# cocowy1/PPMStereo

Hardware: AMD Instinct MI355X
Metric: disparity-px/s (higher is better)
Workload: dtype bf16; 1 GPU; BASELINE config 2: T=5 clip at 320x512, iters=10, hot path only (3-scale cascade from encoder outputs: corr pyramid build + lookup, QAM pick, pick-and-play memory attention, ConvGRU3D update, heads, convex upsample, test_mode=True as PPMStereo.forward_batch_test calls it: predictions[-1] is the output, so the mask head, the convex upsampling and the full-resolution resize run only where their resu; T=5, H=320, W=512, iters=10, parallelism=replicas x1

## Files before the change

### include/ppms.h

```cpp
#ifndef PPMS_H
#define PPMS_H
#include <stdint.h>

#ifdef __cplusplus
extern "C" {
#endif

#define PPMS_OK 0
#define PPMS_EINVAL (-1)
#define PPMS_ELAUNCH (-2)
#define PPMS_ENODEV (-3)

#define PPMS_ABI_VERSION 4

int ppms_version(void);
const char* ppms_last_error(void);
int ppms_device_info(char* name, int name_cap, int* cu_count, int* clock_mhz);

int ppms_corr_build(const float* fmap1, const float* fmap2, float* const pyr[5], int B, int C, int H, int W, void* stream);

int ppms_corr_lookup(const float* const pyr[4], const float* flow, int flow_nhwc, float* out_nchw, void* out_hi, void* out_lo,
                     int out_ld, void* flow_sp_hi, void* flow_sp_lo, int flow_sp_ld, int B, int H, int W, void* stream);

typedef struct ppms_sp {
    void* hi;
    void* lo;
    int32_t ld;
    int32_t c;
} ppms_sp;

enum {
    PPMS_EPI_STORE = 0,
    PPMS_EPI_RESID = 1,
    PPMS_EPI_RH = 2,
    PPMS_EPI_GRU = 3,
    PPMS_EPI_ADDF32 = 4
};
enum { PPMS_ACT_NONE = 0, PPMS_ACT_RELU = 1, PPMS_ACT_GELU = 2, PPMS_ACT_SIGMOID = 3, PPMS_ACT_TANH = 4, PPMS_ACT_ELU1 = 5  };

typedef struct ppms_epilogue {
    int32_t kind, act;
    float scale;
    int32_t n_valid;
    ppms_sp out_sp;
    float* out_f32;
    int32_t out_f32_ld;
    int32_t vt_f16;
    void* out_vt;
    ppms_sp aux_sp;
    const float* aux_f32;
    int32_t aux_f32_ld;
    int32_t pre_f32_ld;
    const float* pre_f32;
} ppms_epilogue;

typedef struct ppms_conv {
    ppms_sp seg[2];
    int32_t nseg;
    int32_t groups;
    const void* w;
    const float* bias;
    int32_t T, H, W;
    int32_t kt, kh, kw;
    int32_t M;
    int32_t m_split;
    int32_t t_halo;
    int32_t lo_zero_from;
    ppms_epilogue epi[2];
} ppms_conv;

int ppms_conv_gemm2(const ppms_conv* desc, const ppms_conv* dev_desc, int wm_hint, void* stream);
int ppms_conv_gemm2_slices(const ppms_conv* desc);
int64_t ppms_conv_gemm2_slice_workspace_bytes(const ppms_conv* desc, int nslice);
int ppms_conv_gemm2_sliced(const ppms_conv* desc, const ppms_conv* dev_desc, int nslice, void* workspace, void* stream);
int ppms_conv_gemm2_ysweep_slices(const ppms_conv* desc);
int ppms_conv_gemm2_ysweep(const ppms_conv* desc, const ppms_conv* dev_desc, int nslice, void* workspace, void* stream);
int ppms_conv_gemm5_applicable(const ppms_conv* desc);
int ppms_conv_gemm5(const ppms_conv* desc, const ppms_conv* dev_desc, int nbt, void* stream);
int ppms_conv_gemm5_slices(const ppms_conv* desc);
int ppms_conv_gemm5_sliced(const ppms_conv* desc, const ppms_conv* dev_desc, int nbt, int nslice, void* workspace, void* stream);
int ppms_conv_gemm6_applicable(const ppms_conv* desc);
int ppms_conv_gemm6(const ppms_conv* desc, const ppms_conv* dev_desc, void* stream);
int ppms_gemm1_applicable(const ppms_conv* desc);
int ppms_gemm1(const ppms_conv* desc, const ppms_conv* dev_desc, int cb_hint, void* stream);
int ppms_conv_stream_applicable(const ppms_conv* desc);
int ppms_conv_stream(const ppms_conv* desc, const ppms_conv* dev_desc, int hint, void* stream);
int ppms_struct_sizes(int* sp, int* epilogue, int* conv);

int ppms_dwconv_gelu(ppms_sp x, ppms_sp y, const float* w, const float* b, int k, int BT, int H, int W, void* stream);
int ppms_flow_patch7(const float* flow_nhwc, ppms_sp patch, int BT, int H, int W, void* stream);
int ppms_unc_tail(ppms_sp x, const float* w, float bias, float* unc, float* partial, int BT, int HW, void* stream);

int ppms_nchw_to_sp(const float* src, ppms_sp dst, int BT, int C, int HW, void* stream);
int ppms_sp_to_nchw(ppms_sp src, float* dst, int BT, int C, int HW, void* stream);
int ppms_nchw_to_nhwc(const float* src, float* dst, int dst_ld, int BT, int C, int HW, void* stream);
int ppms_nhwc_to_nchw(const float* src, int src_ld, float* dst, int BT, int C, int HW, void* stream);
int ppms_f32_to_sp(const float* src, int src_ld, ppms_sp dst, int64_t pixels, void* stream);
int ppms_sp_to_f32(ppms_sp src, float* dst, int dst_ld, int64_t pixels, void* stream);

int ppms_tap_gather_sum(const float* y, int y_ld, const float* bias, float* out, int out_ld, float* accum, int accum_ld, int cout, int kt, int kh,
                        int kw, int T, int H, int W, int t_halo, void* stream);
int ppms_flow_add(float* flow_nhwc, const float* dflow, int dflow_ld, int64_t pixels, void* stream);
int ppms_convex_upsample(const float* flow_nhwc, const float* mask, int mask_ld, float* out, int BT, int H, int W, void* stream);
int ppms_convex_upsample_3d(const float* flow_nhwc, const float* mask, int mask_ld, float* out, int T, int H, int W, int t_halo, void* stream);
int ppms_bilinear(const float* src, float* dst, int N, int C, int H, int W, int OH, int OW, int align_corners, float mul, void* stream);

int ppms_sp_resize_blend(ppms_sp src, ppms_sp dst, int N, int H, int W, int OH, int OW, float a, float b, void* stream);

int ppms_avgpool(const float* src, float* dst, int planes, int H, int W, int k, void* stream);
int ppms_axpby(const float* x, const float* y, float* out, float a, float b, int64_t period, int64_t n, void* stream);
int ppms_ctx_mix(const float* fmap, const float* ctx, float* net, float* inp, int N, int HW, void* stream);

int ppms_img_s2d(const float* img_nchw, ppms_sp dst, int N, int C, int H, int W, int k, void* stream);
int ppms_sp_s2d(ppms_sp src, ppms_sp dst, int N, int H, int W, void* stream);
int64_t ppms_instnorm_workspace_bytes(int N, int HW, int C);
int ppms_instnorm_stats(const float* x, int ld, int N, int HW, int C, float eps, float* stats, void* workspace, void* stream);
int ppms_instnorm_apply(const float* x, int ld, const float* stats, ppms_sp res, int relu, ppms_sp out, int N, int HW, int C, void* stream);

int ppms_dwconv(ppms_sp x, float* y, int ldy, const float* w, const float* b, int k, int N, int H, int W, void* stream);
int ppms_layernorm_any(const float* x, int ld, const float* w, const float* b, float eps, ppms_sp out, int64_t pixels, int C, void* stream);
int64_t ppms_grn_workspace_bytes(int N, int HW, int C);
int ppms_grn(const float* x, int ld, const float* gamma, const float* beta, ppms_sp out, int N, int HW, int C, void* workspace, void* stream);
int ppms_sp_upsample2(ppms_sp src, ppms_sp dst, int N, int H, int W, void* stream);

int ppms_qk_similarity(const float* q, const float* k, int ld, float* pooled, float* sim, int T, int H, int W, void* stream);
int ppms_qk_pool(const float* q, const float* k, int ld, float* pooled, int T, int H, int W, void* stream);
int ppms_qk_cos(const float* pooled, float* sim, int T, int cells, void* stream);
int ppms_qam_select(const float* sim, float* strive, const float* conf_partial, int nblk, int HW, int32_t* sel, float* shat,
                    float* score, int T, void* stream);
int ppms_attn_prep_q(const float* q, int ld, const float* pe, void* qb, int T, int n, void* stream);
int ppms_attn_prep_k(const float* key, int ld, const float* pe, const int32_t* sel, const float* shat, void* kb, int T, int ksel,
                     int n, void* stream);
enum { PPMS_ATTN_P_BF16 = 0, PPMS_ATTN_P_FP16 = 1 };
int ppms_mem_attn(const void* qb, const void* kb, const void* vt, const int32_t* sel, int ksel, float scale, const float* beta,
                  ppms_sp mf, ppms_sp mfg, void* out_bf16, int T, int n, void* split_ws, int frames_per_workgroup, int p_format, void* stream);
int64_t ppms_mem_attn_workspace_bytes(int T, int ksel, int n);

int ppms_pwchain(const void* dev_params, int64_t pixels, void* stream);
int ppms_pwchain_param_bytes(void);

int ppms_time_attn(ppms_sp x, const float* ln_w, const float* ln_b, ppms_sp out, int T, int n, int heads, void* stream);
int ppms_layernorm(const float* x, int ld, const float* w, const float* b, ppms_sp resid, ppms_sp out, int64_t pixels, int C, void* stream);
int64_t ppms_linear_attention_workspace_floats(int T, int n, int heads, int dh);
int ppms_linear_attention(const float* Q, int ldq, const float* K, int ldk, const float* V, int ldv, float* kv_ws, ppms_sp out, int T, int n,
                          int heads, int dh, void* stream);

#ifdef __cplusplus
}
#endif
#endif
```

### ppmstereo_amd/_lib.py

```python
from __future__ import annotations

import ctypes as C
import os
from typing import Optional

import torch

from . import build as _build

c_void_p, c_int, c_float, c_int64 = C.c_void_p, C.c_int, C.c_float, C.c_int64

EPI_STORE, EPI_RESID, EPI_RH, EPI_GRU, EPI_ADDF32 = range(5)
ATTN_P_BF16, ATTN_P_FP16 = 0, 1
ACT_NONE, ACT_RELU, ACT_GELU, ACT_SIGMOID, ACT_TANH, ACT_ELU1 = range(6)


def vt_image(v: torch.Tensor, p_format: int) -> torch.Tensor:
    b = v.to(torch.bfloat16)
    if p_format == ATTN_P_BF16:
        return b.contiguous()
    return b.float().clamp(-65504.0, 65504.0).to(torch.float16).contiguous().view(torch.bfloat16)


def vt_values(vt: torch.Tensor, p_format: int) -> torch.Tensor:
    return vt.float() if p_format == ATTN_P_BF16 else vt.view(torch.float16).float()


class SP(C.Structure):
    _fields_ = [("hi", c_void_p), ("lo", c_void_p), ("ld", C.c_int32), ("c", C.c_int32)]


class Epilogue(C.Structure):
    _fields_ = [("kind", C.c_int32), ("act", C.c_int32), ("scale", c_float), ("n_valid", C.c_int32),
                ("out_sp", SP), ("out_f32", c_void_p), ("out_f32_ld", C.c_int32), ("vt_f16", C.c_int32), ("out_vt", c_void_p),
                ("aux_sp", SP), ("aux_f32", c_void_p), ("aux_f32_ld", C.c_int32), ("pre_f32_ld", C.c_int32),
                ("pre_f32", c_void_p)]


class Conv(C.Structure):
    _fields_ = [("seg", SP * 2), ("nseg", C.c_int32), ("groups", C.c_int32), ("w", c_void_p), ("bias", c_void_p),
                ("T", C.c_int32), ("H", C.c_int32), ("W", C.c_int32),
                ("kt", C.c_int32), ("kh", C.c_int32), ("kw", C.c_int32),
                ("M", C.c_int32), ("m_split", C.c_int32), ("t_halo", C.c_int32), ("lo_zero_from", C.c_int32), ("epi", Epilogue * 2)]


class ChainLayer(C.Structure):
    _fields_ = [("w", c_void_p), ("bias", c_void_p), ("post_s", c_void_p), ("post_t", c_void_p),
                ("M", C.c_int32), ("n_valid", C.c_int32), ("resid", C.c_int32)]


class ChainParams(C.Structure):
    _fields_ = [("inp", SP), ("out", SP), ("layer", ChainLayer * 3), ("nlayers", C.c_int32), ("P", C.c_int64)]


_SIGS = {
    "ppms_version": (c_int, []),
    "ppms_last_error": (C.c_char_p, []),
    "ppms_device_info": (c_int, [C.c_char_p, c_int, C.POINTER(c_int), C.POINTER(c_int)]),
    "ppms_corr_build": (c_int, [c_void_p, c_void_p, C.POINTER(c_void_p), c_int, c_int, c_int, c_int, c_void_p]),
    "ppms_corr_lookup": (c_int, [C.POINTER(c_void_p), c_void_p, c_int, c_void_p, c_void_p, c_void_p, c_int, c_void_p, c_void_p,
                                 c_int, c_int, c_int, c_int, c_void_p]),
    "ppms_conv_gemm2": (c_int, [C.POINTER(Conv), c_void_p, c_int, c_void_p]),
    "ppms_conv_gemm2_slices": (c_int, [C.POINTER(Conv)]),
    "ppms_conv_gemm2_slice_workspace_bytes": (C.c_int64, [C.POINTER(Conv), c_int]),
    "ppms_conv_gemm2_sliced": (c_int, [C.POINTER(Conv), c_void_p, c_int, c_void_p, c_void_p]),
    "ppms_conv_gemm2_ysweep_slices": (c_int, [C.POINTER(Conv)]),
    "ppms_conv_gemm2_ysweep": (c_int, [C.POINTER(Conv), c_void_p, c_int, c_void_p, c_void_p]),
    "ppms_gemm1_applicable": (c_int, [C.POINTER(Conv)]),
    "ppms_gemm1": (c_int, [C.POINTER(Conv), c_void_p, c_int, c_void_p]),
    "ppms_conv_stream_applicable": (c_int, [C.POINTER(Conv)]),
    "ppms_conv_stream": (c_int, [C.POINTER(Conv), c_void_p, c_int, c_void_p]),
    "ppms_conv_gemm5_applicable": (c_int, [C.POINTER(Conv)]),
    "ppms_conv_gemm5": (c_int, [C.POINTER(Conv), c_void_p, c_int, c_void_p]),
    "ppms_conv_gemm6_applicable": (c_int, [C.POINTER(Conv)]),
    "ppms_conv_gemm6": (c_int, [C.POINTER(Conv), c_void_p, c_void_p]),
    "ppms_conv_gemm5_slices": (c_int, [C.POINTER(Conv)]),
    "ppms_conv_gemm5_sliced": (c_int, [C.POINTER(Conv), c_void_p, c_int, c_int, c_void_p, c_void_p]),
    "ppms_struct_sizes": (c_int, [C.POINTER(c_int), C.POINTER(c_int), C.POINTER(c_int)]),
    "ppms_dwconv_gelu": (c_int, [SP, SP, c_void_p, c_void_p, c_int, c_int, c_int, c_int, c_void_p]),
    "ppms_flow_patch7": (c_int, [c_void_p, SP, c_int, c_int, c_int, c_void_p]),
    "ppms_unc_tail": (c_int, [SP, c_void_p, c_float, c_void_p, c_void_p, c_int, c_int, c_void_p]),
    "ppms_nchw_to_sp": (c_int, [c_void_p, SP, c_int, c_int, c_int, c_void_p]),
    "ppms_sp_to_nchw": (c_int, [SP, c_void_p, c_int, c_int, c_int, c_void_p]),
    "ppms_nchw_to_nhwc": (c_int, [c_void_p, c_void_p, c_int, c_int, c_int, c_int, c_void_p]),
    "ppms_nhwc_to_nchw": (c_int, [c_void_p, c_int, c_void_p, c_int, c_int, c_int, c_void_p]),
    "ppms_f32_to_sp": (c_int, [c_void_p, c_int, SP, c_int64, c_void_p]),
    "ppms_sp_to_f32": (c_int, [SP, c_void_p, c_int, c_int64, c_void_p]),
    "ppms_tap_gather_sum": (c_int, [c_void_p, c_int, c_void_p, c_void_p, c_int, c_void_p, c_int, c_int, c_int, c_int, c_int, c_int, c_int, c_int, c_int, c_void_p]),
    "ppms_flow_add": (c_int, [c_void_p, c_void_p, c_int, c_int64, c_void_p]),
    "ppms_convex_upsample": (c_int, [c_void_p, c_void_p, c_int, c_void_p, c_int, c_int, c_int, c_void_p]),
    "ppms_convex_upsample_3d": (c_int, [c_void_p, c_void_p, c_int, c_void_p, c_int, c_int, c_int, c_int, c_void_p]),
    "ppms_bilinear": (c_int, [c_void_p, c_void_p, c_int, c_int, c_int, c_int, c_int, c_int, c_int, c_float, c_void_p]),
    "ppms_sp_resize_blend": (c_int, [SP, SP, c_int, c_int, c_int, c_int, c_int, c_float, c_float, c_void_p]),
    "ppms_avgpool": (c_int, [c_void_p, c_void_p, c_int, c_int, c_int, c_int, c_void_p]),
    "ppms_axpby": (c_int, [c_void_p, c_void_p, c_void_p, c_float, c_float, c_int64, c_int64, c_void_p]),
    "ppms_ctx_mix": (c_int, [c_void_p, c_void_p, c_void_p, c_void_p, c_int, c_int, c_void_p]),
    "ppms_img_s2d": (c_int, [c_void_p, SP, c_int, c_int, c_int, c_int, c_int, c_void_p]),
    "ppms_dwconv": (c_int, [SP, c_void_p, c_int, c_void_p, c_void_p, c_int, c_int, c_int, c_int, c_void_p]),
    "ppms_layernorm_any": (c_int, [c_void_p, c_int, c_void_p, c_void_p, c_float, SP, c_int64, c_int, c_void_p]),
    "ppms_grn_workspace_bytes": (c_int64, [c_int, c_int, c_int]),
    "ppms_grn": (c_int, [c_void_p, c_int, c_void_p, c_void_p, SP, c_int, c_int, c_int, c_void_p, c_void_p]),
    "ppms_sp_upsample2": (c_int, [SP, SP, c_int, c_int, c_int, c_void_p]),
    "ppms_sp_s2d": (c_int, [SP, SP, c_int, c_int, c_int, c_void_p]),
    "ppms_instnorm_workspace_bytes": (c_int64, [c_int, c_int, c_int]),
    "ppms_instnorm_stats": (c_int, [c_void_p, c_int, c_int, c_int, c_int, C.c_float, c_void_p, c_void_p, c_void_p]),
    "ppms_instnorm_apply": (c_int, [c_void_p, c_int, c_void_p, SP, c_int, SP, c_int, c_int, c_int, c_void_p]),
    "ppms_qk_similarity": (c_int, [c_void_p, c_void_p, c_int, c_void_p, c_void_p, c_int, c_int, c_int, c_void_p]),
    "ppms_qk_pool": (c_int, [c_void_p, c_void_p, c_int, c_void_p, c_int, c_int, c_int, c_void_p]),
    "ppms_qk_cos": (c_int, [c_void_p, c_void_p, c_int, c_int, c_void_p]),
    "ppms_qam_select": (c_int, [c_void_p, c_void_p, c_void_p, c_int, c_int, c_void_p, c_void_p, c_void_p, c_int, c_void_p]),
    "ppms_attn_prep_q": (c_int, [c_void_p, c_int, c_void_p, c_void_p, c_int, c_int, c_void_p]),
    "ppms_attn_prep_k": (c_int, [c_void_p, c_int, c_void_p, c_void_p, c_void_p, c_void_p, c_int, c_int, c_int, c_void_p]),
    "ppms_pwchain": (c_int, [c_void_p, c_int64, c_void_p]),
    "ppms_pwchain_param_bytes": (c_int, []),
    "ppms_time_attn": (c_int, [SP, c_void_p, c_void_p, SP, c_int, c_int, c_int, c_void_p]),
    "ppms_layernorm": (c_int, [c_void_p, c_int, c_void_p, c_void_p, SP, SP, c_int64, c_int, c_void_p]),
    "ppms_linear_attention_workspace_floats": (c_int64, [c_int, c_int, c_int, c_int]),
    "ppms_linear_attention": (c_int, [c_void_p, c_int, c_void_p, c_int, c_void_p, c_int, c_void_p, SP, c_int, c_int, c_int, c_int, c_void_p]),
    "ppms_mem_attn": (c_int, [c_void_p, c_void_p, c_void_p, c_void_p, c_int, c_float, c_void_p, SP, SP, c_void_p, c_int, c_int, c_void_p, c_int, c_int, c_void_p]),
    "ppms_mem_attn_workspace_bytes": (c_int64, [c_int, c_int, c_int]),
}
EXPORTS = tuple(_SIGS)

_lib: Optional[C.CDLL] = None


def lib_path() -> str:
    return _build.LIB


def load() -> C.CDLL:
    global _lib
    if _lib is not None:
        return _lib
    try:
        path = _build.build(verbose=not os.path.exists(_build.LIB))
        lib = C.CDLL(path)
    except Exception as exc:
        raise RuntimeError(f"ppmstereo_amd: the HIP library libppms.so is missing and could not be built ({exc}); "
                           "there is no CPU fallback") from exc
    for name, (res, args) in _SIGS.items():
        fn = getattr(lib, name)
        fn.restype, fn.argtypes = res, args
    if lib.ppms_version() != 4:
        raise RuntimeError("ppmstereo_amd: libppms.so ABI version mismatch")
    a, b, c = c_int(), c_int(), c_int()
    lib.ppms_struct_sizes(C.byref(a), C.byref(b), C.byref(c))
    if (a.value, b.value, c.value) != (C.sizeof(SP), C.sizeof(Epilogue), C.sizeof(Conv)):
        raise RuntimeError("ppmstereo_amd: ctypes struct layout differs from include/ppms.h")
    if lib.ppms_pwchain_param_bytes() != C.sizeof(ChainParams):
        raise RuntimeError("ppmstereo_amd: ChainParams layout differs from pwchain.hip")
    _lib = lib
    return lib


def check(rc: int) -> None:
    if rc != 0:
        raise RuntimeError("libppms: " + load().ppms_last_error().decode())


def stream_ptr() -> int:
    return torch.cuda.current_stream().cuda_stream


def require_gpu(*tensors: torch.Tensor) -> None:
    for t in tensors:
        if t is not None and not t.is_cuda:
            raise RuntimeError("ppmstereo_amd ops run on the GPU only (got a CPU tensor); there is no CPU fallback")


def ptr(t: Optional[torch.Tensor]) -> Optional[int]:
    return None if t is None else t.data_ptr()


class SPTensor:

    def __init__(self, pixels: int, channels: int, device, zero: bool = True, before: int = 0, after: int = 0):
        alloc = torch.zeros if zero else torch.empty
        self.data = alloc((2, before + pixels + after, channels), dtype=torch.bfloat16, device=device)
        self.pixels, self.channels, self.before, self.after = pixels, channels, before, after

    def view(self, c0: int = 0, c: Optional[int] = None, all_rows: bool = False) -> SP:
        c = self.channels - c0 if c is None else c
        assert 0 <= c0 and c0 + c <= self.channels
        total = self.before + self.pixels + self.after
        base = self.data.data_ptr() + (0 if all_rows else self.before) * self.channels * 2
        plane = total * self.channels * 2
        return SP(base + c0 * 2, base + plane + c0 * 2, self.channels, c)

    def own(self) -> torch.Tensor:
        return self.data[:, self.before:self.before + self.pixels]

    def to_f32(self, c0: int = 0, c: Optional[int] = None) -> torch.Tensor:
        c = self.channels - c0 if c is None else c
        d = self.own()
        return d[0, :, c0:c0 + c].float() + d[1, :, c0:c0 + c].float()

    def set_f32(self, x: torch.Tensor, c0: int = 0) -> None:
        hi = x.to(torch.bfloat16)
        lo = (x - hi.float()).to(torch.bfloat16)
        d = self.own()
        d[0, :, c0:c0 + x.shape[1]] = hi
        d[1, :, c0:c0 + x.shape[1]] = lo
```

### ppmstereo_amd/build.py

```python
from __future__ import annotations

import fcntl
import hashlib
import os
import shutil
import subprocess
import sys
import tempfile

HERE = os.path.dirname(os.path.abspath(__file__))
ROOT = os.path.dirname(HERE)
CSRC = os.path.join(HERE, "csrc")
LIB = os.path.join(HERE, "libppms.so")
STAMP = LIB + ".stamp"
LOCK = LIB + ".lock"
SOURCES = ["corr.hip", "conv_gemm2.hip", "conv_gemm5.hip", "conv_gemm6.hip", "gemm1.hip", "conv_stream.hip", "small_ops.hip", "encoder_ops.hip", "mem_attn.hip", "attn16.hip", "pwchain.hip"]
HEADERS = ["common.h", "corr_lookup.h", "conv_epilogue.h", "conv5_asm.h", "conv6_asm.h", "attn64_asm.h", os.path.join("..", "..", "include", "ppms.h")]
COMMON = ["--offload-arch=gfx950", "-O3", "-std=c++17", "-fPIC", "-ffp-contract=off", "-I" + os.path.join(ROOT, "include"), "-I" + CSRC]
NO_PK = ["-Xclang", "-target-feature", "-Xclang", "-packed-fp32-ops"]
EXTRA = [x for x in os.environ.get("PPMS_BUILD_DEFINES", "").split() if x]
PACKED_FP32_SOURCES: tuple = tuple(x for x in os.environ.get("PPMS_BUILD_PACKED_FP32", "").split(",") if x)
FLAGS = COMMON + NO_PK + EXTRA


def _digest() -> str:
    h = hashlib.sha256(" ".join(x.replace(ROOT, "$ROOT") for x in FLAGS + list(PACKED_FP32_SOURCES)).encode())
    for f in SOURCES + HEADERS:
        with open(os.path.join(CSRC, f), "rb") as fh:
            h.update(os.path.basename(f).encode() + fh.read())
    return h.hexdigest()


def _fresh(dig: str) -> bool:
    try:
        return os.path.exists(LIB) and open(STAMP).read() == dig
    except OSError:
        return False


def build(force: bool = False, verbose: bool = True) -> str:
    dig = _digest()
    if not force and _fresh(dig):
        return LIB
    hipcc = os.environ.get("HIPCC", "/opt/rocm/bin/hipcc")
    noise = "'-packed-fp32-ops' is not a recognized feature for this target (ignoring feature)"

    def run(cmd):
        if verbose:
            print("[ppmstereo_amd.build]", " ".join(cmd), file=sys.stderr)
        res = subprocess.run(cmd, stderr=subprocess.PIPE, text=True)
        err = "\n".join(ln for ln in res.stderr.splitlines() if noise not in ln)
        if err.strip():
            print(err, file=sys.stderr)
        if res.returncode != 0:
            raise subprocess.CalledProcessError(res.returncode, cmd)

    with open(LOCK, "w") as lock:
        fcntl.flock(lock, fcntl.LOCK_EX)
        try:
            if not force and _fresh(dig):
                return LIB
            tmp = tempfile.mkdtemp(prefix="_build_", dir=HERE)
            try:
                objs = []
                procs = []
                for src in SOURCES:
                    obj = os.path.join(tmp, src.replace(".hip", ".o"))
                    cmd = [hipcc] + (COMMON + EXTRA if src in PACKED_FP32_SOURCES else FLAGS) + ["-c", os.path.join(CSRC, src), "-o", obj]
                    if verbose:
                        print("[ppmstereo_amd.build]", " ".join(cmd), file=sys.stderr)
                    procs.append((cmd, subprocess.Popen(cmd, stderr=subprocess.PIPE, text=True)))
                    objs.append(obj)
                for cmd, pr in procs:
                    _, err = pr.communicate()
                    err = "\n".join(ln for ln in err.splitlines() if noise not in ln)
                    if err.strip():
                        print(err, file=sys.stderr)
                    if pr.returncode != 0:
                        raise subprocess.CalledProcessError(pr.returncode, cmd)
                out = os.path.join(tmp, "libppms.so")
                run([hipcc, "--offload-arch=gfx950", "-shared", "-fPIC"] + objs + ["-o", out])
                stamp = os.path.join(tmp, "stamp")
                with open(stamp, "w") as fh:
                    fh.write(dig)
                if os.path.exists(STAMP):
                    os.remove(STAMP)
                os.replace(out, LIB)
                os.replace(stamp, STAMP)
            finally:
                shutil.rmtree(tmp, ignore_errors=True)
        finally:
            fcntl.flock(lock, fcntl.LOCK_UN)
    return LIB


if __name__ == "__main__":
    print(build(force="--force" in sys.argv))
```

### ppmstereo_amd/csrc/pwchain.hip

```cpp
#include "common.h"

namespace {

constexpr int TP = 128;
constexpr int ROWB = 64;
constexpr int ACT_PLANE = TP * ROWB;
constexpr int ACT_BUF = 4 * ACT_PLANE;
constexpr int W_BLK = 2 * 2 * 64 * 64;

__device__ __forceinline__ int swzp(int row, int chunk) { return row * 64 + ((chunk ^ ((row >> 2) & 3)) << 4); }

struct Layer {
    const void* w;
    const float* bias;
    const float* post_s;
    const float* post_t;
    int M;
    int n_valid;
    int resid;
};

struct ChainParams {
    ppms_sp in, out;
    Layer layer[3];
    int nlayers;
    int64_t P;
};

__global__ __launch_bounds__(256) void pwchain_kernel(const ChainParams* __restrict__ cp) {
    extern __shared__ __attribute__((aligned(16))) char smem[];
    const ChainParams& c = *cp;
    char* bufX = smem;
    char* bufA = smem + ACT_BUF;
    char* wsm = smem + 2 * ACT_BUF;
    const int tid = threadIdx.x, lane = tid & 63, wave = tid >> 6;
    const int r = lane & 31, h = lane >> 5;
    const int64_t p0 = (int64_t)blockIdx.x * TP;

    for (int q = tid; q < TP * 8; q += 256) {
        const int px = q >> 3, ch = q & 7;
        const int64_t pix = p0 + px;
        u32x4 vh = {0, 0, 0, 0}, vl = {0, 0, 0, 0};
        if (pix < c.P) {
            vh = gload16((const bf16_t*)c.in.hi + pix * c.in.ld + ch * 8);
            vl = gload16((const bf16_t*)c.in.lo + pix * c.in.ld + ch * 8);
        }
        const int off = (ch >> 2) * 2 * ACT_PLANE + swzp(px, ch & 3);
        *(u32x4*)(bufX + off) = vh;
        *(u32x4*)(bufX + ACT_PLANE + off) = vl;
    }
    u32x4 wreg[4];
    auto load_w = [&](int l, int mblk) __attribute__((always_inline)) {
        const Layer& Lw = c.layer[l];
        const int mbs = Lw.M / 64;
#pragma unroll
        for (int i = 0; i < 4; ++i) {
            const int q = tid + i * 256;
            const int ks = q >> 9, rem = q & 511;
            wreg[i] = gload16((const char*)Lw.w + ((int64_t)(ks * mbs + mblk) * 512 + rem) * 16);
        }
    };
    load_w(0, 0);
    const char* src = bufX;
    for (int l = 0; l < c.nlayers; ++l) {
        const Layer& L = c.layer[l];
        const bool last = (l == c.nlayers - 1);
        char* dst = (src == bufX) ? bufA : bufX;
        const int mblocks = L.M / 64;
        for (int mblk = 0; mblk < mblocks; ++mblk) {
            __syncthreads();
#pragma unroll
            for (int i = 0; i < 4; ++i) *(u32x4*)(wsm + (tid + i * 256) * 16) = wreg[i];
            if (mblk + 1 < mblocks)
                load_w(l, mblk + 1);
            else if (l + 1 < c.nlayers)
                load_w(l + 1, 0);
            __syncthreads();
            f32x16 acc[2];
            acc[0] = (f32x16){0};
            acc[1] = (f32x16){0};
#pragma unroll
            for (int ks = 0; ks < 2; ++ks) {
#pragma unroll
                for (int k16 = 0; k16 < 2; ++k16) {
                    const int boff = ks * 2 * ACT_PLANE + swzp(wave * 32 + r, 2 * k16 + h);
                    const bf16x8 bh = *(const bf16x8*)(src + boff);
                    const bf16x8 bl = *(const bf16x8*)(src + ACT_PLANE + boff);
#pragma unroll
                    for (int mb = 0; mb < 2; ++mb) {
                        const int aoff = ks * 8192 + swzp(mb * 32 + r, 2 * k16 + h);
                        const bf16x8 ah = *(const bf16x8*)(wsm + aoff);
                        const bf16x8 al = *(const bf16x8*)(wsm + 4096 + aoff);
                        acc[mb] = __builtin_amdgcn_mfma_f32_32x32x16_bf16(al, bh, acc[mb], 0, 0, 0);
                        acc[mb] = __builtin_amdgcn_mfma_f32_32x32x16_bf16(ah, bl, acc[mb], 0, 0, 0);
                        acc[mb] = __builtin_amdgcn_mfma_f32_32x32x16_bf16(ah, bh, acc[mb], 0, 0, 0);
                    }
                }
            }
            const int px = wave * 32 + r;
            const int64_t pix = p0 + px;
#pragma unroll
            for (int mb = 0; mb < 2; ++mb)
#pragma unroll
                for (int g = 0; g < 4; ++g) {
                    const int cl = mb * 32 + 8 * g + 4 * h;
                    const int cg = mblk * 64 + cl;
                    const f32x4 b4 = gld<f32x4>(L.bias + cg);
                    float y[4];
#pragma unroll
                    for (int j = 0; j < 4; ++j) y[j] = acc[mb][4 * g + j] + b4[j];
                    if (L.resid) {
                        const int xo = (cl >> 5) * 2 * ACT_PLANE + swzp(px, (cl & 31) >> 3) + (cl & 7) * 2;
                        const bf16x4 xh = *(const bf16x4*)(bufX + xo), xl = *(const bf16x4*)(bufX + ACT_PLANE + xo);
#pragma unroll
                        for (int j = 0; j < 4; ++j) y[j] += join_bf16(xh[j], xl[j]);
                    }
#pragma unroll
                    for (int j = 0; j < 4; ++j) y[j] = gelu_erf(y[j]);
                    if (L.post_s != nullptr) {
                        const f32x4 s4 = gld<f32x4>(L.post_s + cg), t4 = gld<f32x4>(L.post_t + cg);
#pragma unroll
                        for (int j = 0; j < 4; ++j) y[j] = gelu_erf(y[j] + (y[j] * s4[j] + t4[j]));
                    }
                    bf16x4 oh, ol;
#pragma unroll
                    for (int j = 0; j < 4; ++j) {
                        bf16_t hh = (bf16_t)0.0f, ll = (bf16_t)0.0f;
                        if (cg + j < L.n_valid) split_bf16(y[j], hh, ll);
                        oh[j] = hh;
                        ol[j] = ll;
                    }
                    {
                        const int xo = (cl >> 5) * 2 * ACT_PLANE + swzp(px, (cl & 31) >> 3) + (cl & 7) * 2;
                        *(bf16x4*)(dst + xo) = oh;
                        *(bf16x4*)(dst + ACT_PLANE + xo) = ol;
                    }
                }
            if (last) {
                __syncthreads();
                for (int qd = tid; qd < TP * 16; qd += 256) {
                    const int opx = qd >> 4, plane = (qd >> 3) & 1, ch = qd & 7;
                    const int64_t opix = p0 + opx;
                    const int ocg = mblk * 64 + ch * 8;
                    if (opix < c.P && ocg < L.n_valid) {
                        const u32x4 v = *(const u32x4*)(dst + (ch >> 2) * 2 * ACT_PLANE + plane * ACT_PLANE + swzp(opx, ch & 3));
                        bf16_t* op = (bf16_t*)(plane ? c.out.lo : c.out.hi) + opix * c.out.ld + ocg;
                        if (ocg + 8 <= L.n_valid) {
                            gstore16(op, v);
                        } else {
                            const bf16_t* e = (const bf16_t*)&v;
                            for (int j = 0; j < 8; ++j)
                                if (ocg + j < L.n_valid) gst<bf16_t>(op + j, e[j]);
                        }
                    }
                }
            }
        }
        src = dst;
    }
}

constexpr int TP32 = 32;
constexpr int ACT32_PLANE = TP32 * ROWB;
constexpr int ACT32_BUF = 4 * ACT32_PLANE;
constexpr int W32_MAX = 4 * W_BLK;

__global__ __launch_bounds__(256) void pwchain32_kernel(const ChainParams* __restrict__ cp) {
    extern __shared__ __attribute__((aligned(16))) char smem[];
    const ChainParams& c = *cp;
    char* bufX = smem;
    char* bufA = smem + ACT32_BUF;
    char* wsm = smem + 2 * ACT32_BUF;
    const int tid = threadIdx.x, lane = tid & 63, wave = tid >> 6;
    const int r = lane & 31, h = lane >> 5;
    const int64_t p0 = (int64_t)blockIdx.x * TP32;
    {
        const int px = tid >> 3, ch = tid & 7;
        const int64_t pix = p0 + px;
        u32x4 vh = {0, 0, 0, 0}, vl = {0, 0, 0, 0};
        if (pix < c.P) {
            vh = gload16((const bf16_t*)c.in.hi + pix * c.in.ld + ch * 8);
            vl = gload16((const bf16_t*)c.in.lo + pix * c.in.ld + ch * 8);
        }
        const int off = (ch >> 2) * 2 * ACT32_PLANE + swzp(px, ch & 3);
        *(u32x4*)(bufX + off) = vh;
        *(u32x4*)(bufX + ACT32_PLANE + off) = vl;
    }
    u32x4 wreg[16];
    auto load_w = [&](int l) __attribute__((always_inline)) {
        const Layer& Lw = c.layer[l];
        const int mbs = Lw.M / 64;
#pragma unroll
        for (int mblk = 0; mblk < 4; ++mblk)
            if (mblk < mbs) {
#pragma unroll
                for (int i = 0; i < 4; ++i) {
                    const int q = tid + i * 256;
                    const int ks = q >> 9, rem = q & 511;
                    wreg[mblk * 4 + i] = gload16((const char*)Lw.w + ((int64_t)(ks * mbs + mblk) * 512 + rem) * 16);
                }
            }
    };
    load_w(0);
    const char* src = bufX;
    for (int l = 0; l < c.nlayers; ++l) {
        const Layer& L = c.layer[l];
        const bool last = (l == c.nlayers - 1);
        char* dst = (src == bufX) ? bufA : bufX;
        const int mbs = L.M / 64, nrb = L.M / 32;
        __syncthreads();
#pragma unroll
        for (int mblk = 0; mblk < 4; ++mblk)
            if (mblk < mbs) {
#pragma unroll
                for (int i = 0; i < 4; ++i) *(u32x4*)(wsm + mblk * W_BLK + (tid + i * 256) * 16) = wreg[mblk * 4 + i];
            }
        if (l + 1 < c.nlayers) load_w(l + 1);
        __syncthreads();
        bf16x4 keep_h[2][4], keep_l[2][4];
#pragma unroll
        for (int it = 0; it < 2; ++it) {
            const int rb = wave + 4 * it;
            if (rb >= nrb) continue;
            const int mblk = rb >> 1, mb = rb & 1;
            f32x16 acc = (f32x16){0};
#pragma unroll
            for (int ks = 0; ks < 2; ++ks)
#pragma unroll
                for (int k16 = 0; k16 < 2; ++k16) {
                    const int boff = ks * 2 * ACT32_PLANE + swzp(r, 2 * k16 + h);
                    const bf16x8 bh = *(const bf16x8*)(src + boff), bl = *(const bf16x8*)(src + ACT32_PLANE + boff);
                    const int aoff = mblk * W_BLK + ks * 8192 + swzp(mb * 32 + r, 2 * k16 + h);
                    const bf16x8 ah = *(const bf16x8*)(wsm + aoff), al = *(const bf16x8*)(wsm + 4096 + aoff);
                    acc = __builtin_amdgcn_mfma_f32_32x32x16_bf16(al, bh, acc, 0, 0, 0);
                    acc = __builtin_amdgcn_mfma_f32_32x32x16_bf16(ah, bl, acc, 0, 0, 0);
                    acc = __builtin_amdgcn_mfma_f32_32x32x16_bf16(ah, bh, acc, 0, 0, 0);
                }
#pragma unroll
            for (int g = 0; g < 4; ++g) {
                const int cl = mb * 32 + 8 * g + 4 * h;
                const int cg = mblk * 64 + cl;
                const f32x4 b4 = gld<f32x4>(L.bias + cg);
                float y[4];
#pragma unroll
                for (int j = 0; j < 4; ++j) y[j] = acc[4 * g + j] + b4[j];
                const int xo = (cl >> 5) * 2 * ACT32_PLANE + swzp(r, (cl & 31) >> 3) + (cl & 7) * 2;
                if (L.resid) {
                    const bf16x4 xh = *(const bf16x4*)(bufX + xo), xl = *(const bf16x4*)(bufX + ACT32_PLANE + xo);
#pragma unroll
                    for (int j = 0; j < 4; ++j) y[j] += join_bf16(xh[j], xl[j]);
                }
#pragma unroll
                for (int j = 0; j < 4; ++j) y[j] = gelu_erf(y[j]);
                if (L.post_s != nullptr) {
                    const f32x4 s4 = gld<f32x4>(L.post_s + cg), t4 = gld<f32x4>(L.post_t + cg);
#pragma unroll
                    for (int j = 0; j < 4; ++j) y[j] = gelu_erf(y[j] + (y[j] * s4[j] + t4[j]));
                }
                bf16x4 oh, ol;
#pragma unroll
                for (int j = 0; j < 4; ++j) {
                    bf16_t hh = (bf16_t)0.0f, ll = (bf16_t)0.0f;
                    if (cg + j < L.n_valid) split_bf16(y[j], hh, ll);
                    oh[j] = hh;
                    ol[j] = ll;
                }
                if (last) {
                    keep_h[it][g] = oh;
                    keep_l[it][g] = ol;
                } else {
                    *(bf16x4*)(dst + xo) = oh;
                    *(bf16x4*)(dst + ACT32_PLANE + xo) = ol;
                }
            }
        }
        if (last) {
            __syncthreads();
            const int rowb = L.M * 2 + 16;
#pragma unroll
            for (int it = 0; it < 2; ++it) {
                const int rb = wave + 4 * it;
                if (rb >= nrb) continue;
#pragma unroll
                for (int g = 0; g < 4; ++g) {
                    const int cg = rb * 32 + 8 * g + 4 * h;
                    *(bf16x4*)(wsm + r * rowb + cg * 2) = keep_h[it][g];
                    *(bf16x4*)(wsm + TP32 * rowb + r * rowb + cg * 2) = keep_l[it][g];
                }
            }
            __syncthreads();
            const int cpr = L.M / 8;
            for (int qd = tid; qd < TP32 * 2 * cpr; qd += 256) {
                const int plane = qd / (TP32 * cpr), rem = qd - plane * TP32 * cpr;
                const int opx = rem / cpr, ch = rem - opx * cpr;
                const int64_t opix = p0 + opx;
                const int ocg = ch * 8;
                if (opix < c.P && ocg < L.n_valid) {
                    const u32x4 v = *(const u32x4*)(wsm + plane * TP32 * rowb + opx * rowb + ocg * 2);
                    bf16_t* op = (bf16_t*)(plane ? c.out.lo : c.out.hi) + opix * c.out.ld + ocg;
                    if (ocg + 8 <= L.n_valid) {
                        gstore16(op, v);
                    } else {
                        const bf16_t* e = (const bf16_t*)&v;
                        for (int j = 0; j < 8; ++j)
                            if (ocg + j < L.n_valid) gst<bf16_t>(op + j, e[j]);
                    }
                }
            }
        }
        src = dst;
    }
}

}

static int pwchain_launch(const void* dev_params, int64_t pixels, void* stream) {
    constexpr size_t lds = 2 * ACT_BUF + W_BLK;
    constexpr size_t lds32 = 2 * ACT32_BUF + W32_MAX;
    static ppms_device_once once;
    once.run([] {
        (void)hipFuncSetAttribute((const void*)pwchain_kernel, hipFuncAttributeMaxDynamicSharedMemorySize, (int)(2 * ACT_BUF + W_BLK));
        (void)hipFuncSetAttribute((const void*)pwchain32_kernel, hipFuncAttributeMaxDynamicSharedMemorySize, (int)(2 * ACT32_BUF + W32_MAX));
    });
    if (pixels <= 16384) {
        hipLaunchKernelGGL(pwchain32_kernel, dim3(ceil_div(pixels, TP32)), dim3(256), lds32, (hipStream_t)stream, (const ChainParams*)dev_params);
        return ppms_check_launch("pwchain");
    }
    hipLaunchKernelGGL(pwchain_kernel, dim3(ceil_div(pixels, TP)), dim3(256), lds, (hipStream_t)stream, (const ChainParams*)dev_params);
    return ppms_check_launch("pwchain");
}

extern "C" int ppms_pwchain(const void* dev_params, int64_t pixels, void* stream) {
    PPMS_REQUIRE(dev_params != nullptr && pixels > 0, "pwchain: bad arguments");
    return pwchain_launch(dev_params, pixels, stream);
}

extern "C" int ppms_pwchain_param_bytes(void) { return (int)sizeof(ChainParams); }
```

### ppmstereo_amd/engine.py

```python
from __future__ import annotations

import ctypes as C
import math
from typing import Dict, List, Optional

import torch

from . import _lib as L
from . import packing as _packing
from .convplan import (ALL_KERNELS, CONV2, CONV2_SWEPT, CONV6, KERNEL_TIMING, TUNING, ConvOp, PwChain, TimedCall,
                       attn_p_format, conv_desc, epilogue, pack_conv, plan_conv)

TOP_K = 5


def temporal_pe(T: int, channels: int) -> torch.Tensor:
    pos = torch.arange(T)
    pos = pos / pos[-1] * 1.0
    pos = pos.unsqueeze(1)
    div = 1.0 / (10000.0 ** (torch.arange(0, channels, 2).float() / channels))
    ang = pos * div
    pe = torch.zeros(T, channels)
    pe[:, 0::2] = torch.sin(ang)
    pe[:, 1::2] = torch.cos(ang)
    return pe


def softmax_scale(c: int = 128) -> float:
    return c ** -0.5 * math.log(2 * c, 12000)


class PackedBlock:

    def __init__(self, sd: Dict[str, torch.Tensor], device):
        g = lambda k: sd[k].detach().to(device=device, dtype=torch.float32)
        self.w: Dict[str, dict] = {}

        def put(name, weight, bias, segs, seg_pad=None, cout_map=None, m_pad=None, kernels=ALL_KERNELS):
            self.w[name] = pack_conv(weight, bias, segs, seg_pad, cout_map, m_pad, kernels)

        e = "encoder."
        put("init0", g(e + "init_conv.0.weight"), g(e + "init_conv.0.bias"), [128])
        put("init2", g(e + "init_conv.2.weight"), g(e + "init_conv.2.bias"), [64])
        c1 = e + "convc1."
        put("ffn1_0", g(c1 + "ffn1.0.weight"), g(c1 + "ffn1.0.bias"), [36], [64], kernels=(CONV2,))
        put("ffn1_2", g(c1 + "ffn1.2.weight"), g(c1 + "ffn1.2.bias"), [54], [64], kernels=(CONV2,))
        put("pw", g(c1 + "pw.weight"), g(c1 + "pw.bias"), [36], [64], kernels=(CONV2,))
        put("ffn2_0", g(c1 + "ffn2.0.weight"), g(c1 + "ffn2.0.bias"), [36], [64], kernels=(CONV2,))
        put("ffn2_2", g(c1 + "ffn2.2.weight"), g(c1 + "ffn2.2.bias"), [54], [64], kernels=(CONV2,))
        self.dw = []
        for i, k in ((0, 1), (1, 7)):
            w = torch.zeros(64, k * k, device=device)
            b = torch.zeros(64, device=device)
            w[:36] = g(c1 + f"conv_list.{i}.weight").reshape(36, k * k)
            b[:36] = g(c1 + f"conv_list.{i}.bias")
            self.dw.append((w.contiguous(), b.contiguous(), k))
        put("convc2", g(e + "convc2.weight"), g(e + "convc2.bias"), [256])
        wf1 = g(e + "convf1.weight").permute(0, 2, 3, 1).reshape(128, 98, 1, 1)
        put("convf1", wf1, g(e + "convf1.bias"), [98], [128])
        put("convf2", g(e + "convf2.weight"), g(e + "convf2.bias"), [128])
        put("final", g(e + "final_conv.weight"), g(e + "final_conv.bias"), [320], None, list(range(126)) + list(range(128, 192)), 192)
        put("to_v", g("aggregator.to_v.weight"), None, [128])
        put("unc0", g("uncertainty.0.weight"), g("uncertainty.0.bias"), [128, 128])
        self.unc2_w = g("uncertainty.2.weight").reshape(128).contiguous()
        self.unc2_b = float(sd["uncertainty.2.bias"].detach().float().cpu().item())
        gr = "gru."
        cat = lambda a, b: torch.cat([g(a), g(b)], 0)
        put("zr1_0", cat(gr + "convz1.0.weight", gr + "convr1.0.weight"), cat(gr + "convz1.0.bias", gr + "convr1.0.bias"), [128, 384])
        put("z1_2", g(gr + "convz1.2.weight"), g(gr + "convz1.2.bias"), [128])
        put("r1_2", g(gr + "convr1.2.weight"), g(gr + "convr1.2.bias"), [128])
        self.w["zr1_2"] = {CONV6: _packing.pack_conv6_grouped([g(gr + "convz1.2.weight"), g(gr + "convr1.2.weight")], [g(gr + "convz1.2.bias"), g(gr + "convr1.2.bias")], 128)}
        put("q1", g(gr + "convq1.weight"), g(gr + "convq1.bias"), [128, 384])
        for n in ("2", "3"):
            put("zr" + n, cat(gr + f"convz{n}.weight", gr + f"convr{n}.weight"), cat(gr + f"convz{n}.bias", gr + f"convr{n}.bias"), [128, 384])
            put("q" + n, g(gr + f"convq{n}.weight"), g(gr + f"convq{n}.bias"), [128, 384])
        self.hoist = "time_attn.temporal_fc.weight" not in sd
        if self.hoist:
            for name in ("zr1_0", "q1", "zr2", "q2", "zr3", "q3"):
                if name.startswith("zr"):
                    n_ = name[2:].replace("1_0", "1.0")
                    wt, bs = cat(gr + f"convz{n_}.weight", gr + f"convr{n_}.weight"), cat(gr + f"convz{n_}.bias", gr + f"convr{n_}.bias")
                else:
                    wt, bs = g(gr + f"convq{name[1:]}.weight"), g(gr + f"convq{name[1:]}.bias")
                w_h = torch.cat([wt[:, :128], wt[:, 256:]], 1).contiguous()
                put(name + "_i", wt[:, 128:256].contiguous(), bs, [128], kernels=ALL_KERNELS - {CONV2_SWEPT})
                put(name + "_h", w_h, None, [128, 256])
                beta = float(sd["aggregator.beta"].detach().double().reshape(-1)[0])
                wd = wt.double()
                w_x = torch.cat([wd[:, :128], wd[:, 256:384] + wd[:, 384:], beta * wd[:, 384:]], 1).float().contiguous()
                put(name + "_x", w_x, None, [128, 256])
        put("fh1", g("flow_head.conv1.weight"), g("flow_head.conv1.bias"), [128])
        w2 = g("flow_head.conv2.weight")
        put("fh2", w2.permute(2, 3, 4, 0, 1).reshape(54, 256, 1, 1, 1).contiguous(), None, [256])
        self.fh2_bias = g("flow_head.conv2.bias").contiguous()
        self.convex_3d = "mask_3d.0.weight" in sd
        mk = "mask_3d." if self.convex_3d else "mask_2d."
        put("m1", g(mk + "0.weight"), g(mk + "0.bias"), [128])
        put("m2", g(mk + "2.weight"), g(mk + "2.bias"), [256])
        self.mask_ch = 432 if self.convex_3d else 144
        self.beta = g("aggregator.beta").contiguous()
        self.attn = None
        if "time_attn.temporal_fc.weight" in sd:
            self.attn = {k: g(k) for k in sd if k.startswith("time_attn.") or k.startswith("space_attn.")}
            lin = lambda k: g(k)[:, :, None, None]
            ta, sa = "time_attn.", "space_attn.encoder_layer."
            w_fc, w_pj = g(ta + "temporal_fc.weight").double(), g(ta + "temporal_attn.proj.weight").double()
            w_ta = (w_fc @ w_pj).float().contiguous()
            b_ta = (w_fc @ g(ta + "temporal_attn.proj.bias").double() + g(ta + "temporal_fc.bias").double()).float().contiguous()
            put("ta_fc", w_ta[:, :, None, None], b_ta, [384])
            put("sa_qkv", torch.cat([lin(sa + "q_proj.weight"), lin(sa + "k_proj.weight"), lin(sa + "v_proj.weight")], 0), None, [384])
            put("sa_merge", lin(sa + "merge.weight"), None, [384])
            put("sa_mlp0", lin(sa + "mlp.0.weight"), None, [384, 384])
            put("sa_mlp2", lin(sa + "mlp.2.weight"), None, [768])
            self.ln = {k: (g(p_ + ".weight").contiguous(), g(p_ + ".bias").contiguous())
                       for k, p_ in (("ta", ta + "temporal_norm1"), ("n1", sa + "norm1"), ("n2", sa + "norm2"))}


class ScaleEngine:

    def __init__(self, pk: PackedBlock, T: int, h: int, w: int, device, shard=None):
        if shard is not None and shard.world == 1 and not getattr(shard, "force_comm", False):
            shard = None
        if shard is not None and T != shard.f:
            raise ValueError(f"sharded engine: {T} local frames, the shard holds {shard.f}")
        self.shard = shard
        self.Tg = Tg = T if shard is None else shard.T
        self.f0 = 0 if shard is None else shard.lo
        self.halo = 0 if shard is None else shard.HALO
        if Tg > 64:
            raise NotImplementedError("more than 64 frames per window")
        self.pk, self.T, self.h, self.w = pk, T, h, w
        self.n = n = h * w
        self.P = P = T * h * w
        self.dev = device
        self.ksel = min(TOP_K, Tg)
        hp = self.halo * n
        sp = lambda c: L.SPTensor(P, c, device, before=hp, after=hp)
        f32 = lambda *s: torch.zeros(*s, dtype=torch.float32, device=device)
        self.CORR, self.T1, self.C1, self.C2 = sp(64), sp(64), sp(64), sp(64)
        self.COR256, self.CF, self.PATCH, self.FLO1 = sp(256), [sp(320), sp(320)], sp(128), sp(128)
        self.X, self.VAL, self.U1 = sp(384), sp(128), sp(128)
        self.XA = sp(384) if pk.attn is not None else self.X
        if pk.attn is not None:
            self.XT, self.MSG, self.MSGN, self.H1 = sp(384), sp(384), sp(384), sp(768)
            self.O1 = L.SPTensor(P, 384, device, before=self.f0 * n, after=(Tg - self.f0 - T) * n)
            self.XG = self.X if shard is None else L.SPTensor(Tg * n, 384, device)
            self.QKF, self.VF, self.M2, self.M3 = f32(P, 768), f32(P, 384), f32(P, 384), f32(P, 384)
            self.KVWS = f32(int(L.load().ppms_linear_attention_workspace_floats(T, n, 8, 48)))
        self.Hb = [sp(128), sp(128), sp(128)]
        self.ZT, self.RT, self.RH, self.FH1, self.M1 = sp(128), sp(128), sp(128), sp(256), sp(256)
        self.Z, self.MASK, self.QK = f32(P, 128), f32(P, pk.mask_ch), f32(P, 256)
        self._FLOW_full, self._FH2Y_full = f32(P + 2 * hp, 2), f32(P + 2 * hp, 64)
        self.FLOW, self.FH2Y = self._FLOW_full[hp:hp + P], self._FH2Y_full[hp:hp + P]
        self.DFLOW = f32(P, 4)
        if pk.hoist:
            self.PRE = {k: torch.empty(P, m, dtype=torch.float32, device=device) for k, m in
                        (("zr1_0", 256), ("q1", 128), ("zr2", 256), ("q2", 128), ("zr3", 256), ("q3", 128))}
            self._pre_stream, self._ev_pre, self._pre_pending = torch.cuda.Stream(device=device), torch.cuda.Event(), False
        self.attn_p = attn_p_format()
        self.VT = torch.zeros(T, 128, n, dtype=torch.bfloat16, device=device)
        self.VTG = self.VT if shard is None else torch.zeros(Tg, 128, n, dtype=torch.bfloat16, device=device)
        self.KG = None if shard is None else f32(Tg * n, 128)
        self.QB = torch.zeros(T, n, 128, dtype=torch.bfloat16, device=device)
        self.KB = torch.zeros(T, self.ksel, n, 128, dtype=torch.bfloat16, device=device)
        self.ATT_WS = torch.empty(int(L.load().ppms_mem_attn_workspace_bytes(T, self.ksel, n)), dtype=torch.uint8, device=device)
        self.nblk = (n + 255) // 256
        self.UNC, self.PART = f32(P), f32(T, self.nblk)
        self.PARTG = self.PART if shard is None else f32(Tg, self.nblk)
        self.SIM, self.STRIVE, self.SCORE = f32(Tg, Tg), f32(Tg, Tg), f32(Tg, Tg)
        self.SEL = torch.zeros(Tg, 5, dtype=torch.int32, device=device)
        self.SHAT = f32(Tg, 5)
        self.cells = max(1, (h // 4) * (w // 4))
        self.POOL = f32(2, T, self.cells)
        self.POOLG = self.POOL if shard is None else f32(2, Tg, self.cells)
        self.PE = temporal_pe(Tg, 128).to(device)
        self.FLOW_OUT = f32(T, 2, 4 * h, 4 * w)
        self.scale = softmax_scale(128)
        self.parity = 0
        self.have_mhs = False
        self.lib = L.load()
        self._ev, self._ev_i = None, 0
        self._xa_halo = None
        self._x_hid = False
        self.hbm = {"corr_lookup": TimedCall(self._lookup), "attn_prep_k": TimedCall(self._prep_k), "convex_upsample": TimedCall(self._upsample)}
        self._side = torch.cuda.Stream(device=device)
        self._ev_fork, self._ev_join = torch.cuda.Event(), torch.cuda.Event()
        self._build_descriptors()

    def _halo_sp(self, tensors, k: int, async_op: bool = False):
        if self.shard is None:
            return None
        if isinstance(tensors, L.SPTensor):
            tensors = [tensors]
        fr = self.T + 2 * self.halo
        return self.shard.halo_many([(t.data[p].view(fr, self.n, t.channels), k) for t in tensors for p in (0, 1)], async_op)

    def _halo_f32(self, full: torch.Tensor, k: int):
        if self.shard is not None:
            self.shard.halo(full.view(self.T + 2 * self.halo, self.n, full.shape[1]), k)

    def _conv(self, packs, segs: List[L.SP], k3, epi0: L.Epilogue, epi1: Optional[L.Epilogue] = None, m_split: int = 0, keep=(),
              lo_zero_from: int = 0) -> ConvOp:
        d = conv_desc(segs, (self.T, self.h, self.w), k3, epi0, epi1, m_split, self.halo if k3[0] > 1 else 0, lo_zero_from)
        return plan_conv(d, self.pk.w[packs] if isinstance(packs, str) else packs, keep, device=self.dev)

    def _build_descriptors(self):
        E, X, H = epilogue, self.X, self.Hb
        k1, k3 = (1, 1, 1), (1, 3, 3)
        inp, mf, mfg = X.view(0, 128), X.view(128, 128), X.view(256, 128)
        self.op: Dict[str, object] = {}
        o = self.op
        self._qk_ops: Dict[int, ConvOp] = {}
        o["init0"] = self._conv("init0", [inp], k3, E(act=L.ACT_RELU, n_valid=64, out_sp=self.ZT.view(0, 64)))
        w = {k: self.pk.w[k][CONV2] for k in ("ffn1_0", "ffn1_2", "pw", "ffn2_0", "ffn2_2")}
        (w1, b1, _), (w7, b7, _) = self.pk.dw
        dw1 = (w1.reshape(64).contiguous(), b1)
        o["chainA"] = PwChain(self.CORR.view(), self.C2.view(), [(w["ffn1_0"], 54, False, None), (w["ffn1_2"], 36, True, dw1)], self.P, [dw1[0]],
                             device=self.dev)
        o["chainB"] = PwChain(self.C1.view(), self.COR256.view(), [(w["pw"], 36, True, None), (w["ffn2_0"], 54, False, None),
                                                                   (w["ffn2_2"], 256, False, None)], self.P, [], device=self.dev)
        o["dw7"] = TimedCall(lambda: L.check(self.lib.ppms_dwconv_gelu(self.C2.view(0, 40), self.C1.view(0, 40), w7.data_ptr(), b7.data_ptr(), 7,
                                                                        self.T, self.h, self.w, L.stream_ptr())))
        o["convf1"] = self._conv("convf1", [self.PATCH.view()], k1, E(act=L.ACT_RELU, n_valid=128, out_sp=self.FLO1.view()))
        for par in (0, 1):
            cf, cf_next = self.CF[par], self.CF[1 - par]
            o[f"init2_{par}"] = self._conv("init2", [self.ZT.view(0, 64)], k3, E(n_valid=64, out_sp=cf.view(256, 64)))
            o[f"convc2_{par}"] = self._conv("convc2", [self.COR256.view()], k3, E(act=L.ACT_RELU, n_valid=192, out_sp=cf.view(0, 192)))
            o[f"convf2_{par}"] = self._conv("convf2", [self.FLO1.view()], k3, E(act=L.ACT_RELU, n_valid=64, out_sp=cf.view(192, 64)))
            o[f"final_{par}"] = self._conv("final", [cf.view()], k3, E(act=L.ACT_RELU, n_valid=126, out_sp=mf),
                                           E(act=L.ACT_RELU, n_valid=64, out_sp=cf_next.view(256, 64)), m_split=128)
        o["to_v"] = self._conv("to_v", [mf], k1, E(n_valid=128, out_sp=self.VAL.view(), out_vt=self.VT, vt_f16=self.attn_p))
        o["unc0"] = self._conv("unc0", [H[0].view(), self.VAL.view()], k3, E(act=L.ACT_RELU, n_valid=128, out_sp=self.U1.view()))
        if self.pk.attn is not None:
            o["ta_fc"] = self._conv("ta_fc", [self.O1.view()], k1, E(L.EPI_RESID, n_valid=384, out_sp=self.XT.view(), aux_sp=X.view()))
            o["sa_qkv"] = self._conv("sa_qkv", [self.XT.view()], k1, E(act=L.ACT_ELU1, n_valid=768, out_f32=self.QKF, out_f32_ld=768),
                                     E(scale=1.0 / self.n, n_valid=384, out_f32=self.VF, out_f32_ld=384), m_split=768)
            o["sa_merge"] = self._conv("sa_merge", [self.MSG.view()], k1, E(n_valid=384, out_f32=self.M2, out_f32_ld=384))
            o["sa_mlp0"] = self._conv("sa_mlp0", [self.XT.view(), self.MSGN.view()], k1, E(act=L.ACT_RELU, n_valid=768, out_sp=self.H1.view()))
            o["sa_mlp2"] = self._conv("sa_mlp2", [self.H1.view()], k1, E(n_valid=384, out_f32=self.M3, out_f32_ld=384))
        x_all = self.XA.view()
        hoist = self.pk.hoist
        if hoist:
            x_all = X.view(128, 256)
            for k, kk in (("zr1_0", (1, 1, 15)), ("q1", (1, 1, 5)), ("zr2", (1, 5, 1)), ("q2", (1, 5, 1)), ("zr3", (5, 1, 1)), ("q3", (5, 1, 1))):
                m = self.PRE[k].shape[1]
                o["pre_" + k] = self._conv(k + "_i", [inp], kk, E(n_valid=m, out_f32=self.PRE[k], out_f32_ld=m))
        pre = lambda k, off=0: dict(pre_f32=self.PRE[k], pre_off=off) if hoist else {}
        o["z1_2"] = self._conv("z1_2", [self.ZT.view()], (1, 1, 5), E(act=L.ACT_SIGMOID, n_valid=128, out_f32=self.Z, out_f32_ld=128))
        o["r1_2"] = self._conv("r1_2", [self.RT.view()], (1, 1, 5), E(L.EPI_RH, n_valid=128, out_sp=self.RH.view(), aux_sp=H[0].view()))
        if TUNING["conv6_grouped"]:
            dg = conv_desc([self.ZT.view(), self.RT.view()], (self.T, self.h, self.w), (1, 1, 5), o["z1_2"].desc.epi[0], o["r1_2"].desc.epi[0], m_split=128)
            dg.groups = 2
            op = plan_conv(dg, self.pk.w["zr1_2"], [self.ZT, self.RT, self.Z, self.RH, H[0]], device=self.dev)
            if op is not None:
                o["zr1_2"] = op
        self.hid_mode = hoist
        for tag, sfx, lz in ((("", "_h", 0), ("_x", "_x", 256)) if hoist else (("", "", 0),)):
            o["zr1_0" + tag] = self._conv("zr1_0" + sfx, [H[0].view(), x_all], (1, 1, 15), E(act=L.ACT_GELU, n_valid=128, out_sp=self.ZT.view(), **pre("zr1_0")),
                                          E(act=L.ACT_GELU, n_valid=128, out_sp=self.RT.view(), **pre("zr1_0", 128)), m_split=128, lo_zero_from=lz)
            o["q1" + tag] = self._conv("q1" + sfx, [self.RH.view(), x_all], (1, 1, 5),
                                       E(L.EPI_GRU, n_valid=128, out_sp=H[1].view(), aux_sp=H[0].view(), aux_f32=self.Z, aux_f32_ld=128, **pre("q1")), lo_zero_from=lz)
            for n, kk, src, dst in (("2", (1, 5, 1), 1, 2), ("3", (5, 1, 1), 2, 0)):
                o["zr" + n + tag] = self._conv("zr" + n + sfx, [H[src].view(), x_all], kk,
                                               E(act=L.ACT_SIGMOID, n_valid=128, out_f32=self.Z, out_f32_ld=128, **pre("zr" + n)),
                                               E(L.EPI_RH, n_valid=128, out_sp=self.RH.view(), aux_sp=H[src].view(), **pre("zr" + n, 128)), m_split=128,
                                               lo_zero_from=lz)
                o["q" + n + tag] = self._conv("q" + n + sfx, [self.RH.view(), x_all], kk,
                                              E(L.EPI_GRU, n_valid=128, out_sp=H[dst].view(), aux_sp=H[src].view(), aux_f32=self.Z, aux_f32_ld=128,
                                                **pre("q" + n)), lo_zero_from=lz)
        o["fh1"] = self._conv("fh1", [H[0].view()], (3, 3, 3), E(act=L.ACT_RELU, n_valid=256, out_sp=self.FH1.view()))
        o["fh2"] = self._conv("fh2", [self.FH1.view()], k1, E(n_valid=54, out_f32=self.FH2Y, out_f32_ld=64))
        o["m1"] = self._conv("m1", [H[0].view()], (3, 3, 3) if self.pk.convex_3d else k3, E(act=L.ACT_RELU, n_valid=256, out_sp=self.M1.view()))
        o["m2"] = self._conv("m2", [self.M1.view()], k1, E(scale=0.25, n_valid=self.pk.mask_ch, out_f32=self.MASK, out_f32_ld=self.pk.mask_ch))

    def _s(self):
        return L.stream_ptr()

    def load_nchw(self, x: torch.Tensor, dst: L.SP):
        x = x.contiguous().float()
        L.require_gpu(x)
        L.check(self.lib.ppms_nchw_to_sp(x.data_ptr(), dst, x.shape[0], x.shape[1], x.shape[2] * x.shape[3], self._s()))

    def store_nchw(self, src: L.SP, c: int) -> torch.Tensor:
        out = torch.empty(self.T, c, self.h, self.w, dtype=torch.float32, device=self.dev)
        L.check(self.lib.ppms_sp_to_nchw(src, out.data_ptr(), self.T, c, self.n, self._s()))
        return out

    def _drain_xa_halo(self):
        if self._xa_halo is not None:
            self._xa_halo.wait()
            self._xa_halo = None

    def set_inp(self, inp: torch.Tensor):
        self._drain_xa_halo()
        self.load_nchw(inp, self.X.view(0, 128))
        self._halo_sp(self.X, 2)
        if self.pk.hoist:
            self._ev_fork.record()
            self._pre_stream.wait_event(self._ev_fork)
            with torch.cuda.stream(self._pre_stream):
                for k in ("zr1_0", "q1", "zr2", "q2", "zr3", "q3"):
                    self.op["pre_" + k]()
                self._ev_pre.record()
            self._pre_pending = True

    def set_net(self, net: torch.Tensor):
        self.load_nchw(net, self.Hb[0].view())

    def set_mf(self, mf: torch.Tensor):
        self.load_nchw(mf, self.X.view(128, 128))

    def set_mfg(self, mfg: torch.Tensor):
        self.load_nchw(mfg, self.X.view(256, 128))
        self._x_hid = False

    def set_flow(self, flow: torch.Tensor):
        f = flow.contiguous().float()
        L.require_gpu(f)
        L.check(self.lib.ppms_nchw_to_nhwc(f.data_ptr(), self.FLOW.data_ptr(), 2, self.T, 2, self.n, self._s()))

    def set_mhs(self, mhs: Optional[torch.Tensor]):
        self.parity = 0
        self.have_mhs = mhs is not None
        if mhs is not None:
            self.load_nchw(mhs, self.CF[self.parity].view(256, 64))

    def net_view(self) -> L.SP:
        return self.Hb[0].view()

    def mhs_view(self) -> L.SP:
        return self.CF[self.parity].view(256, 64)

    def UNC_local(self) -> torch.Tensor:
        return self.UNC

    def get_net(self):
        return self.store_nchw(self.Hb[0].view(), 128)

    def get_mhs(self):
        return self.store_nchw(self.CF[self.parity].view(256, 64), 64)

    def get_mf(self):
        return self.store_nchw(self.X.view(128, 128), 128)

    def get_mfg(self):
        if self._x_hid:
            mfg = self.X.to_f32(128, 128) + self.pk.beta * self.X.to_f32(256, 128)
            return mfg.reshape(self.T, self.h, self.w, 128).permute(0, 3, 1, 2).contiguous()
        return self.store_nchw(self.X.view(256, 128), 128)

    def get_value(self):
        return self.store_nchw(self.VAL.view(), 128)

    def get_flow(self):
        out = torch.empty(self.T, 2, self.h, self.w, dtype=torch.float32, device=self.dev)
        L.check(self.lib.ppms_nhwc_to_nchw(self.FLOW.data_ptr(), 2, out.data_ptr(), self.T, 2, self.n, self._s()))
        return out

    def get_dflow(self):
        out = torch.empty(self.T, 2, self.h, self.w, dtype=torch.float32, device=self.dev)
        L.check(self.lib.ppms_nhwc_to_nchw(self.DFLOW.data_ptr(), 4, out.data_ptr(), self.T, 2, self.n, self._s()))
        return out

    def get_mask(self):
        mc = self.pk.mask_ch
        out = torch.empty(self.T, mc, self.h, self.w, dtype=torch.float32, device=self.dev)
        L.check(self.lib.ppms_nhwc_to_nchw(self.MASK.data_ptr(), mc, out.data_ptr(), self.T, mc, self.n, self._s()))
        return out

    def get_unc(self):
        return self.UNC.view(self.T, 1, self.h, self.w).clone()

    def begin(self, pyramid: List[torch.Tensor], qk_pack):
        self._drain_xa_halo()
        self.pyr = pyramid
        self.pyr_ptrs = (C.c_void_p * 4)(*[p.data_ptr() for p in pyramid[:4]])
        self.qk_op(qk_pack)()
        s = self._s()
        pe_local = self.PE.data_ptr() + self.f0 * 128 * 4
        L.check(self.lib.ppms_attn_prep_q(self.QK.data_ptr(), 256, pe_local, self.QB.data_ptr(), self.T, self.n, s))
        L.check(self.lib.ppms_qk_pool(self.QK.data_ptr(), self.QK.data_ptr() + 128 * 4, 256, self.POOL.data_ptr(), self.T, self.h, self.w, s))
        if self.shard is not None:
            g, _ = self.shard.all_gather(self.POOL.permute(1, 0, 2).contiguous())
            self.POOLG.copy_(g.permute(1, 0, 2))
            self.shard.all_gather(self.QK[:, 128:].contiguous(), out=self.KG)
        L.check(self.lib.ppms_qk_cos(self.POOLG.data_ptr(), self.SIM.data_ptr(), self.Tg, self.cells, s))
        self.STRIVE.fill_(1.0)

    def qk_op(self, qk_pack) -> ConvOp:
        key = qk_pack[CONV2][0].data_ptr()
        if key not in self._qk_ops:
            self._qk_ops[key] = self._conv(qk_pack, [self.X.view(0, 128)], (1, 1, 1), epilogue(n_valid=256, out_f32=self.QK, out_f32_ld=256))
        return self._qk_ops[key]

    def lookup(self):
        self.hbm["corr_lookup"]()

    def _lookup(self):
        X = self.X
        fl = X.view(254, 2)
        L.check(self.lib.ppms_corr_lookup(self.pyr_ptrs, self.FLOW.data_ptr(), 1, None, self.CORR.view().hi, self.CORR.view().lo, 64,
                                          fl.hi, fl.lo, 384, self.T, self.h, self.w, self._s()))

    def hbm_bytes(self) -> Dict[str, float]:
        T, n, w = self.T, self.n, self.w
        return dict(corr_lookup=T * n * (4 * 10 * 4 + 36 * 4 + 8.0), attn_prep_k=self.Tg * n * 128 * 4.0 + T * self.ksel * n * 128 * 2.0,
                    convex_upsample=T * n * (self.pk.mask_ch + 2) * 4.0 + T * 16 * n * 2 * 4.0,
                    corr_build=2 * 256 * T * n * 4.0 + 1.9375 * T * n * w * 4.0)

    def _fork(self):
        self._ev_fork.record()
        self._side.wait_event(self._ev_fork)
        return torch.cuda.stream(self._side)

    def _join(self):
        self._ev_join.record(self._side)
        torch.cuda.current_stream().wait_event(self._ev_join)

    def motion_and_value(self):
        o, par = self.op, self.parity
        with self._fork():
            L.check(self.lib.ppms_flow_patch7(self.FLOW.data_ptr(), self.PATCH.view(), self.T, self.h, self.w, self._s()))
            o["convf1"]()
            o[f"convf2_{par}"]()
        if not self.have_mhs:
            o["init0"]()
            o[f"init2_{par}"]()
            self.have_mhs = True
        o["chainA"]()
        o["dw7"]()
        o["chainB"]()
        o[f"convc2_{par}"]()
        self._join()
        o[f"final_{par}"]()
        self.parity = 1 - par
        o["to_v"]()

    def uncertainty(self):
        self.op["unc0"]()
        L.check(self.lib.ppms_unc_tail(self.U1.view(), self.pk.unc2_w.data_ptr(), self.pk.unc2_b, self.UNC.data_ptr(), self.PART.data_ptr(),
                                       self.T, self.n, self._s()))

    def pick(self):
        if self.shard is not None:
            self.shard.gather_many([(self.VT, self.VTG), (self.PART, self.PARTG)])
        L.check(self.lib.ppms_qam_select(self.SIM.data_ptr(), self.STRIVE.data_ptr(), self.PARTG.data_ptr(), self.nblk, self.n, self.SEL.data_ptr(),
                                         self.SHAT.data_ptr(), self.SCORE.data_ptr(), self.Tg, self._s()))

    def attend(self, out_bf16: Optional[torch.Tensor] = None):
        s = self._s()
        sel = self.SEL.data_ptr() + self.f0 * 5 * 4
        shat = self.SHAT.data_ptr() + self.f0 * 5 * 4
        if self.shard is None:
            key, key_ld = self.QK.data_ptr() + 128 * 4, 256
        else:
            key, key_ld = self.KG.data_ptr(), 128
        self._prep_k_args = (key, key_ld, sel, shat)
        self.hbm["attn_prep_k"]()
        ev = None
        if KERNEL_TIMING["on"] and self._ev is not None and self._ev_i < len(self._ev):
            ev = self._ev[self._ev_i]
            self._ev_i += 1
            ev[0].record()
        mf_in = L.SP(None, None, 0, 0) if self.hid_mode else self.X.view(128, 128)
        L.check(self.lib.ppms_mem_attn(self.QB.data_ptr(), self.KB.data_ptr(), self.VTG.data_ptr(), sel, self.ksel, self.scale,
                                       self.pk.beta.data_ptr(), mf_in, self.X.view(256, 128), L.ptr(out_bf16), self.T, self.n,
                                       self.ATT_WS.data_ptr(), 0, self.attn_p, s))
        self._x_hid = self.hid_mode
        if ev is not None:
            ev[1].record()
        if self.shard is not None and self.pk.attn is None:
            self._drain_xa_halo()
            self._xa_halo = self._halo_sp(self.XA, 2, async_op=True)

    def conv_ops(self, version: Optional[int] = None):
        return {k: v for k, v in self.op.items() if isinstance(v, ConvOp) and (version is None or v.version == version)}

    def conv_family_ops(self):
        fam = {k: v for k, v in self.op.items() if isinstance(v, (ConvOp, PwChain, TimedCall))}
        fam.update({f"to_qk_{i}": v for i, v in enumerate(self._qk_ops.values())})
        return fam

    def attn_redo_count(self):
        if self.n % 64:
            return 0, 0
        flags = self.ATT_WS.view(torch.int32)[self.T * self.ksel * self.n * 130:]
        g64 = (self.n + 255) // 256
        used = self.T * self.ksel * g64
        f = flags[:used * 2:2]
        torch.cuda.synchronize()
        return int(used), int((f != 0).sum().item())

    def enable_attn_timing(self, launches: int):
        self._ev = [(torch.cuda.Event(enable_timing=True), torch.cuda.Event(enable_timing=True)) for _ in range(launches)]
        self._ev_i = 0

    def attn_times_ms(self):
        torch.cuda.synchronize()
        return [a.elapsed_time(b) for a, b in self._ev[:self._ev_i]]

    def block16_attention(self):
        o, s, lib, ln = self.op, self._s(), self.lib, self.pk.ln
        none_sp = L.SP(None, None, 0, 0)
        if self.shard is not None:
            self.shard.gather_many([(self.X.own()[pl].view(self.T, self.n, 384), self.XG.data[pl].view(self.Tg, self.n, 384)) for pl in (0, 1)])
        L.check(lib.ppms_time_attn(self.XG.view(all_rows=True), ln["ta"][0].data_ptr(), ln["ta"][1].data_ptr(), self.O1.view(all_rows=True),
                                   self.Tg, self.n, 8, s))
        o["ta_fc"]()
        o["sa_qkv"]()
        L.check(lib.ppms_linear_attention(self.QKF.data_ptr(), 768, self.QKF.data_ptr() + 384 * 4, 768, self.VF.data_ptr(), 384,
                                          self.KVWS.data_ptr(), self.MSG.view(), self.T, self.n, 8, 48, s))
        o["sa_merge"]()
        L.check(lib.ppms_layernorm(self.M2.data_ptr(), 384, ln["n1"][0].data_ptr(), ln["n1"][1].data_ptr(), none_sp, self.MSGN.view(), self.P, 384, s))
        o["sa_mlp0"]()
        o["sa_mlp2"]()
        L.check(lib.ppms_layernorm(self.M3.data_ptr(), 384, ln["n2"][0].data_ptr(), ln["n2"][1].data_ptr(), self.XT.view(), self.XA.view(), self.P, 384, s))

    def update(self, need_mask: bool = True):
        o = self.op
        if self.pk.attn is not None:
            self.block16_attention()
            if self.shard is not None:
                self._xa_halo = self._halo_sp(self.XA, 2, async_op=True)
        if self.pk.hoist and self._pre_pending:
            torch.cuda.current_stream().wait_event(self._ev_pre)
            self._pre_pending = False
        tag = "_x" if self._x_hid else ""
        o["zr1_0" + tag]()
        if "zr1_2" in o:
            o["zr1_2"]()
        else:
            with self._fork():
                o["r1_2"]()
            o["z1_2"]()
            self._join()
        for k in ("q1", "zr2", "q2"):
            o[k + tag]()
        if self.shard is not None:
            self._halo_sp(self.Hb[2], 2)
            if self._xa_halo is not None:
                self._xa_halo.wait()
                self._xa_halo = None
            else:
                self._halo_sp(self.XA, 2)
        o["zr3" + tag]()
        self._halo_sp(self.RH, 2)
        o["q3" + tag]()
        self._halo_sp(self.Hb[0], 1)
        if need_mask:
            with self._fork():
                o["m1"]()
                o["m2"]()
        o["fh1"]()
        o["fh2"]()
        self._halo_f32(self._FH2Y_full, 1)
        L.check(self.lib.ppms_tap_gather_sum(self.FH2Y.data_ptr(), 64, self.pk.fh2_bias.data_ptr(), self.DFLOW.data_ptr(), 4, self.FLOW.data_ptr(), 2,
                                             2, 3, 3, 3, self.T, self.h, self.w, self.halo, self._s()))
        if need_mask:
            self._join()

    def upsample(self) -> torch.Tensor:
        self.hbm["convex_upsample"]()
        return self.FLOW_OUT

    def _prep_k(self):
        key, key_ld, sel, shat = self._prep_k_args
        L.check(self.lib.ppms_attn_prep_k(key, key_ld, self.PE.data_ptr(), sel, shat, self.KB.data_ptr(), self.T, self.ksel, self.n, self._s()))

    def _upsample(self):
        if self.pk.convex_3d:
            self._halo_f32(self._FLOW_full, 1)
            L.check(self.lib.ppms_convex_upsample_3d(self.FLOW.data_ptr(), self.MASK.data_ptr(), self.pk.mask_ch, self.FLOW_OUT.data_ptr(), self.T,
                                                     self.h, self.w, self.halo, self._s()))
        else:
            L.check(self.lib.ppms_convex_upsample(self.FLOW.data_ptr(), self.MASK.data_ptr(), self.pk.mask_ch, self.FLOW_OUT.data_ptr(), self.T,
                                                  self.h, self.w, self._s()))

    def iterate(self, need_up: bool = True):
        self.lookup()
        self.motion_and_value()
        self.uncertainty()
        self.pick()
        self.attend()
        self.update(need_mask=need_up)
        return self.upsample() if need_up else None


def bilinear(x: torch.Tensor, size, align_corners: bool, mul: float = 1.0) -> torch.Tensor:
    x = x.contiguous().float()
    L.require_gpu(x)
    N, Cc, H, W = x.shape
    out = torch.empty(N, Cc, size[0], size[1], dtype=torch.float32, device=x.device)
    L.check(L.load().ppms_bilinear(x.data_ptr(), out.data_ptr(), N, Cc, H, W, size[0], size[1], int(align_corners), mul, L.stream_ptr()))
    return out
```

### ppmstereo_amd/ppmstereo.py

```python
from __future__ import annotations

import math
import warnings
from typing import Dict, List, Optional

import torch
import torch.nn as nn

from . import _lib as L
from .corr import CorrBlock1D
from .engine import bilinear
from .update import Attention_qk, SequenceUpdateBlock3D


def interp(x: torch.Tensor, size) -> torch.Tensor:
    return bilinear(x, (int(size[0]), int(size[1])), True)


def convex_upsample(flow: torch.Tensor, mask: torch.Tensor, rate: int = 4) -> torch.Tensor:
    if rate != 4:
        raise NotImplementedError("convex_upsample: rate 4 only")
    L.require_gpu(flow, mask)
    N, _, H, W = flow.shape
    lib, s = L.load(), L.stream_ptr()
    f = torch.empty(N * H * W, 2, dtype=torch.float32, device=flow.device)
    m = torch.empty(N * H * W, 144, dtype=torch.float32, device=flow.device)
    fc, mc = flow.contiguous().float(), mask.contiguous().float()
    L.check(lib.ppms_nchw_to_nhwc(fc.data_ptr(), f.data_ptr(), 2, N, 2, H * W, s))
    L.check(lib.ppms_nchw_to_nhwc(mc.data_ptr(), m.data_ptr(), 144, N, 144, H * W, s))
    out = torch.empty(N, 2, 4 * H, 4 * W, dtype=torch.float32, device=flow.device)
    L.check(lib.ppms_convex_upsample(f.data_ptr(), m.data_ptr(), 144, out.data_ptr(), N, H, W, s))
    return out


def _run_iterations(eng, iters: int, isc: int, t: int, h: int, w: int, predictions: List, uncertainties: List, emit: str = "all"):
    flow_out = None
    for it in range(iters):
        flow_out = eng.iterate(need_up=(emit == "all" or it + 1 == iters))
        if emit == "none" or (emit == "last" and it + 1 < iters):
            continue
        unc_up = bilinear(eng.UNC_local().view(t, 1, h, w), (4 * isc * h, 4 * isc * w), False)
        if isc > 1:
            flow_up = bilinear(flow_out[:, :1], (isc * 4 * h, isc * 4 * w), True, float(isc))
        else:
            flow_up = flow_out[:, :1].clone()
        predictions.append(flow_up)
        uncertainties.append(unc_up)
    return flow_out


def convex_upsample_3d(flow: torch.Tensor, mask: torch.Tensor, rate: int, T: int) -> torch.Tensor:
    if rate != 4:
        raise NotImplementedError("convex_upsample_3d: rate 4 only")
    L.require_gpu(flow, mask)
    N, _, H, W = flow.shape
    if N != T:
        raise NotImplementedError("convex_upsample_3d: batch size 1 (N == T)")
    lib, s = L.load(), L.stream_ptr()
    f = torch.empty(N * H * W, 2, dtype=torch.float32, device=flow.device)
    m = torch.empty(N * H * W, 432, dtype=torch.float32, device=flow.device)
    fc, mc = flow.contiguous().float(), mask.contiguous().float()
    L.check(lib.ppms_nchw_to_nhwc(fc.data_ptr(), f.data_ptr(), 2, N, 2, H * W, s))
    L.check(lib.ppms_nchw_to_nhwc(mc.data_ptr(), m.data_ptr(), 432, N, 432, H * W, s))
    out = torch.empty(N, 2, 4 * H, 4 * W, dtype=torch.float32, device=flow.device)
    L.check(lib.ppms_convex_upsample_3d(f.data_ptr(), m.data_ptr(), 432, out.data_ptr(), T, H, W, 0, s))
    return out


def forward_update_block(self, image1, update_block: SequenceUpdateBlock3D, corr_fn: CorrBlock1D, flow: torch.Tensor, net: torch.Tensor,
                         inp: torch.Tensor, motion_hidden_state: Optional[torch.Tensor], attn_block: Attention_qk, predictions: List,
                         uncertainties: List, iters: int, interp_scale: float, t: int):
    L.require_gpu(flow, net, inp)
    bt, c, h, w = inp.shape
    if bt % t:
        raise RuntimeError(f"forward_update_block: {bt} frames do not divide into clips of t = {t}")
    if bt != t:
        return _forward_update_block_batched(update_block, corr_fn, flow, net, inp, motion_hidden_state, attn_block, predictions, uncertainties,
                                             iters, interp_scale, t)
    if c != 128:
        raise RuntimeError("forward_update_block: 128 context channels expected")
    if int(interp_scale) not in (1, 2, 4):
        raise NotImplementedError("interp_scale must be 4, 2 or 1 (the reference's only live branches)")
    if t == 1:
        warnings.warn("PPMStereo with a single frame produces NaN disparities (reference behaviour, T must be >= 2)")
    isc = int(interp_scale)
    with torch.cuda.device(inp.device):
        eng = update_block.engine(t, h, w, inp.device)
        eng.set_inp(inp)
        eng.set_net(net)
        eng.set_flow(flow)
        eng.set_mhs(motion_hidden_state)
        eng.begin(corr_fn.levels, attn_block.packed(inp.device))
        flow_out = _run_iterations(eng, iters, isc, t, h, w, predictions, uncertainties)
        return flow_out.clone(), eng.get_net(), eng.get_mhs()


def _forward_update_block_batched(update_block, corr_fn, flow, net, inp, motion_hidden_state, attn_block, predictions, uncertainties, iters,
                                  interp_scale, t: int):
    bt, c, h, w = inp.shape
    b = bt // t
    if c != 128 or int(interp_scale) not in (1, 2, 4):
        raise RuntimeError("forward_update_block: 128 context channels and interp_scale 4, 2 or 1 expected")
    if t == 1:
        warnings.warn("PPMStereo with a single frame produces NaN disparities (reference behaviour, T must be >= 2)")
    isc, dev = int(interp_scale), inp.device
    rows = t * h * w
    with torch.cuda.device(dev):
        engs = []
        for bi in range(b):
            sl = slice(bi * t, (bi + 1) * t)
            eng = update_block.engine(t, h, w, dev, slot=bi)
            eng.set_inp(inp[sl]), eng.set_net(net[sl]), eng.set_flow(flow[sl])
            eng.set_mhs(None if motion_hidden_state is None else motion_hidden_state[sl])
            eng.begin([lv[bi * rows:(bi + 1) * rows] for lv in corr_fn.levels], attn_block.packed(dev))
            engs.append(eng)
        k = engs[0].ksel
        flow_out = None
        for _ in range(iters):
            for eng in engs:
                eng.lookup(), eng.motion_and_value(), eng.uncertainty(), eng.pick()
            picked = [eng.SCORE.gather(1, eng.SEL[:, :k].long()) for eng in engs]
            mean_all = torch.stack([x.sum(1) for x in picked]).sum(0) / float(b * k)
            outs, uncs = [], []
            for eng, x in zip(engs, picked):
                eng.SHAT[:, :k] = x / mean_all[:, None]
                eng.attend(), eng.update(need_mask=True)
                outs.append(eng.upsample().clone())
                uncs.append(eng.UNC_local().view(t, 1, h, w).clone())
            flow_out = torch.cat(outs)
            unc = torch.cat(uncs)
            uncertainties.append(bilinear(unc, (4 * isc * h, 4 * isc * w), False))
            predictions.append(bilinear(flow_out[:, :1], (isc * 4 * h, isc * 4 * w), True, float(isc)) if isc > 1 else flow_out[:, :1].clone())
        return flow_out, torch.cat([e.get_net() for e in engs]), torch.cat([e.get_mhs() for e in engs])


class ClipPipeline:

    def __init__(self, device=None, small_priority: int = 0):
        device = torch.device("cuda", torch.cuda.current_device()) if device is None else torch.device(device)
        self.device = device
        self.small = torch.cuda.Stream(device=device, priority=small_priority)
        self.large = torch.cuda.Stream(device=device)
        self.consumed: Optional[torch.cuda.Event] = None
        self.last: Optional[torch.cuda.Event] = None
        self.serial = False
        self.done_events: List[torch.cuda.Event] = []
        self.record_done = False

        self._results: List[torch.Tensor] = []

    def wait(self, handle: Optional[torch.cuda.Event] = None):
        ev = self.last if handle is None else handle
        cur = torch.cuda.current_stream(self.device)
        if ev is not None:
            cur.wait_event(ev)
        for t in self._results:
            t.record_stream(cur)
        self._results.clear()


class PPMStereoHotPath(nn.Module):

    def __init__(self, max_disp: int = 192, mixed_precision: bool = False, num_frames: int = 5,
                 attention_type: Optional[str] = "self_stereo_temporal_update_time_update_space", use_3d_update_block: bool = True,
                 different_update_blocks: bool = True, use_convex_3d: bool = False, init_flow: bool = False):
        super().__init__()
        if not (use_3d_update_block and different_update_blocks) or init_flow:
            raise NotImplementedError("supported configurations: models/ppm_stereo_model.py:27-33 (use_3d_update_block=True, "
                                      "different_update_blocks=True, init_flow=False) with use_convex_3d False or True (train.py / test.py default)")
        self.hidden_dim = self.context_dim = 128
        self.mixed_precision = mixed_precision
        self.use_convex_3d = bool(use_convex_3d)
        self.num_frames = num_frames
        self.att = nn.ModuleList([Attention_qk(num_heads=1, dim_head=128) for _ in range(3)])
        c3 = self.use_convex_3d
        self.update_block08 = SequenceUpdateBlock3D(hidden_dim=128, cor_planes=36, mask_size=4, use_convex_3d=c3)
        self.update_block16 = SequenceUpdateBlock3D(hidden_dim=128, cor_planes=36, mask_size=4, use_convex_3d=c3, attention_type=attention_type)
        self.update_block04 = SequenceUpdateBlock3D(hidden_dim=128, cor_planes=36, mask_size=4, use_convex_3d=c3)

    forward_update_block = forward_update_block

    def convex_upsample(self, flow, mask, rate: int = 4):
        return convex_upsample(flow, mask, rate)

    def convex_upsample_3d(self, flow, mask, rate: int, T: int):
        return convex_upsample_3d(flow, mask, rate, T)

    def zero_init(self, fmap: torch.Tensor) -> torch.Tensor:
        N, _, H, W = fmap.shape
        return torch.zeros(N, 2, H, W, dtype=torch.float32, device=fmap.device)

    def load_hot_path_weights(self, weights: Dict[str, Dict[str, torch.Tensor]]):
        for tag in ("update_block16", "update_block08", "update_block04"):
            getattr(self, tag).load_state_dict(weights[tag], strict=True)
        for i in range(3):
            self.att[i].load_state_dict(weights[f"att.{i}"], strict=True)
        return self

    @torch.no_grad()
    def cascade(self, feats: Dict[str, torch.Tensor], iters: int, t: int, predictions: Optional[list] = None,
                uncertainties: Optional[list] = None, shard=None, test_mode: bool = False, pipeline: Optional[ClipPipeline] = None):
        if iters < 2:
            raise ValueError(f"cascade: iters={iters}; the 1/16 and 1/8 scales run iters // 2 iterations each (ppmstereo.py:708,744) and need at least one")
        preds = [] if predictions is None else predictions
        uncs = [] if uncertainties is None else uncertainties
        dev = feats["f1_16"].device
        tl = feats["f1_16"].shape[0]
        if shard is None and tl != t:
            if tl % t or pipeline is not None:
                raise RuntimeError(f"cascade: {tl} frames do not divide into clips of t = {t} (or a pipeline was given for a batch)")
            return self._cascade_batched(feats, iters, t, preds, uncs)
        if t == 1:
            warnings.warn("PPMStereo with a single frame produces NaN disparities (reference behaviour, T must be >= 2)")
        lib = L.load()
        with torch.cuda.device(dev):
            caller = torch.cuda.current_stream()
            if pipeline is not None:
                pipeline.small.wait_stream(caller)
                if pipeline.serial and pipeline.last is not None:
                    pipeline.small.wait_event(pipeline.last)
            prev, fo = None, None
            for s_, blk, ai, n_it, isc in ((16, self.update_block16, 0, iters // 2, 4), (8, self.update_block08, 1, iters // 2, 2),
                                          (4, self.update_block04, 2, iters, 1)):
                f1, f2 = feats[f"f1_{s_}"], feats[f"f2_{s_}"]
                h, w = f1.shape[2:]
                stream = caller if pipeline is None else (pipeline.large if s_ == 4 else pipeline.small)
                if pipeline is not None:
                    if s_ == 8 and pipeline.consumed is not None:
                        stream.wait_event(pipeline.consumed)
                    if s_ == 4:
                        stream.wait_stream(pipeline.small)
                    for k in (f"f1_{s_}", f"f2_{s_}", f"net_{s_}", f"inp_{s_}"):
                        feats[k].record_stream(stream)
                with torch.cuda.stream(stream):
                    eng = blk.engine(tl, h, w, dev, shard)
                    eng.set_inp(feats[f"inp_{s_}"])
                    eng.set_net(feats[f"net_{s_}"])
                    if prev is None:
                        eng.set_flow(self.zero_init(f1))
                        eng.set_mhs(None)
                    else:
                        ph, pw = prev.h, prev.w
                        eng.set_flow(bilinear(fo, (h, w), True, -(h / fo.shape[2])))
                        eng.parity, eng.have_mhs = 0, True
                        L.check(lib.ppms_sp_resize_blend(prev.mhs_view(), eng.mhs_view(), tl, ph, pw, 2 * ph, 2 * pw, 0.0, 1.0, L.stream_ptr()))
                        L.check(lib.ppms_sp_resize_blend(prev.net_view(), eng.net_view(), tl, ph, pw, 2 * ph, 2 * pw, 0.5, 0.5, L.stream_ptr()))
                    if pipeline is not None and s_ == 4:
                        pipeline.consumed = torch.cuda.Event()
                        pipeline.consumed.record()
                    eng.begin(CorrBlock1D(f1, f2).levels, self.att[ai].packed(dev))
                    fo = _run_iterations(eng, n_it, isc, tl, h, w, preds, uncs, "all" if not test_mode else ("last" if s_ == 4 else "none"))
                    prev = eng
            if pipeline is not None:
                pipeline.last = torch.cuda.Event(enable_timing=pipeline.record_done)
                pipeline.last.record(pipeline.large)
                if pipeline.record_done:
                    pipeline.done_events.append(pipeline.last)
                pipeline._results += [preds[-1], uncs[-1]]
                del pipeline._results[:-16]
            return preds[-1], uncs[-1]


def _cascade_batched(self, feats, iters: int, t: int, preds: list, uncs: list):
    f16 = feats["f1_16"]
    fo, net16, mhs16 = self.forward_update_block(None, self.update_block16, CorrBlock1D(f16, feats["f2_16"]), self.zero_init(f16), feats["net_16"],
                                                 feats["inp_16"], None, self.att[0], preds, uncs, iters // 2, 4, t)
    nets, mhs = {16: net16}, {16: mhs16}
    for s_, blk, ai, n_it, isc in ((8, self.update_block08, 1, iters // 2, 2), (4, self.update_block04, 2, iters, 1)):
        f1, f2 = feats[f"f1_{s_}"], feats[f"f2_{s_}"]
        h, w = f1.shape[2:]
        flow = bilinear(fo, (h, w), True, -(h / fo.shape[2]))
        m_up = bilinear(mhs[2 * s_], (h, w), True)
        net = (feats[f"net_{s_}"] + bilinear(nets[2 * s_], (h, w), True)) / 2.0
        fo, nets[s_], mhs[s_] = self.forward_update_block(None, blk, CorrBlock1D(f1, f2), flow, net, feats[f"inp_{s_}"], m_up, self.att[ai],
                                                          preds, uncs, n_it, isc, t)
    return preds[-1], uncs[-1]


PPMStereoHotPath._cascade_batched = _cascade_batched


def position_encoding_sine(d_model: int, h: int, w: int) -> torch.Tensor:
    pe = torch.zeros((d_model, h, w))
    y_position = torch.ones((h, w)).cumsum(0).float().unsqueeze(0)
    x_position = torch.ones((h, w)).cumsum(1).float().unsqueeze(0)
    div_term = torch.exp(torch.arange(0, d_model // 2, 2).float() * (-math.log(10000.0) / (d_model // 2)))[:, None, None]
    pe[0::4, :, :] = torch.sin(x_position * div_term)
    pe[1::4, :, :] = torch.cos(x_position * div_term)
    pe[2::4, :, :] = torch.sin(y_position * div_term)
    pe[3::4, :, :] = torch.cos(y_position * div_term)
    return pe


class InputPadder:

    def __init__(self, dims, mode: str = "sintel", divis_by: int = 8):
        self.ht, self.wd = int(dims[-2]), int(dims[-1])
        extra_h, extra_w = -self.ht % divis_by, -self.wd % divis_by
        left, top = extra_w // 2, (extra_h // 2 if mode == "sintel" else 0)
        self._pad = [left, extra_w - left, top, extra_h - top]

    def pad(self, *inputs):
        for x in inputs:
            if x.ndim != 4:
                raise ValueError(f"InputPadder.pad: 4-D tensors expected, got {tuple(x.shape)}")
        if not any(self._pad):
            return list(inputs)
        return [torch.nn.functional.pad(x, self._pad, mode="replicate") for x in inputs]

    def unpad(self, x):
        if x.ndim != 4:
            raise ValueError(f"InputPadder.unpad: 4-D tensor expected, got {tuple(x.shape)}")
        left, right, top, bottom = self._pad
        return x[..., top:x.shape[-2] - bottom, left:x.shape[-1] - right]


class PPMStereo(PPMStereoHotPath):

    WRAPPER_CONFIG = dict(mixed_precision=True, num_frames=5, attention_type="self_stereo_temporal_update_time_update_space",
                          use_3d_update_block=True, different_update_blocks=True)

    @classmethod
    def shipped(cls, **overrides):
        return cls(**{**cls.WRAPPER_CONFIG, **overrides})

    def __init__(self, max_disp: int = 192, mixed_precision: bool = False, num_frames: int = 5, attention_type: Optional[str] = None,
                 use_3d_update_block: bool = False, different_update_blocks: bool = False, use_convex_3d: bool = False, init_flow: bool = False,
                 *, fnet=None, cnet=None, sst="auto"):
        if not (use_3d_update_block and different_update_blocks):
            raise NotImplementedError("PPMStereo: the gfx950 implementation serves the released configuration, models/ppm_stereo_model.py:27-33 -- "
                                      "use_3d_update_block=True, different_update_blocks=True (PPMStereo.shipped() / PPMStereo.WRAPPER_CONFIG); the "
                                      "2-D update block selected by the reference's constructor defaults is outside the hot path")
        super().__init__(max_disp, mixed_precision, num_frames, attention_type, use_3d_update_block, different_update_blocks, use_convex_3d, init_flow)
        at = attention_type
        if isinstance(sst, str) and sst == "auto":
            sst = None
            if at is not None and ("self_stereo" in at or "temporal" in at):
                if not ("self_stereo" in at and "temporal" in at):
                    raise NotImplementedError("SST block: attention types with both 'self_stereo' and 'temporal' (the shipped model) or neither")
                from .sst import SSTBlock
                blk = SSTBlock(dim=256, num_frames=self.num_frames)
                self.time_embed = blk.time_embed
                self.time_attn_blocks, self.self_attn_blocks, self.cross_attn_blocks = blk.time_attn_blocks, blk.self_attn_blocks, blk.cross_attn_blocks
                object.__setattr__(self, "_sst_impl", blk)
                sst = blk
        if fnet is None:
            from .encoder import BasicEncoder
            fnet = BasicEncoder(output_dim=256, norm_fn="instance")
        if cnet is None:
            from .cnet import Feature
            cnet = Feature(model_name="tiny", output_dim=256)
        self.fnet, self.cnet = (None if fnet is False else fnet), (None if cnet is False else cnet)
        object.__setattr__(self, "sst", sst)
        ref_order = ["fnet", "cnet", "att", "update_block08", "update_block16", "update_block04", "time_attn_blocks", "self_attn_blocks", "cross_attn_blocks"]
        mods = self._modules
        for k in [k for k in ref_order if k in mods] + [k for k in list(mods) if k not in ref_order]:
            mods[k] = mods.pop(k)
        self.dim = 256
        self._pe_cache: Dict[tuple, torch.Tensor] = {}
        self.parallel_encoders = True
        self._enc_streams: Dict[int, torch.cuda.Stream] = {}

    def _encoder_stream(self, device) -> torch.cuda.Stream:
        idx = torch.device(device).index or 0
        if idx not in self._enc_streams:
            self._enc_streams[idx] = torch.cuda.Stream(device=device)
        return self._enc_streams[idx]

    def load_state_dict(self, sd, strict: bool = True, **kw):
        r = super().load_state_dict(sd, strict=strict, **kw)
        for m in (self.fnet, self.cnet, getattr(self, "_sst_impl", None)):
            if hasattr(m, "invalidate"):
                m.invalidate()
        return r

    def _pe(self, h: int, w: int, device) -> torch.Tensor:
        key = (h, w, str(device))
        if key not in self._pe_cache:
            self._pe_cache[key] = position_encoding_sine(self.dim, h, w).to(device).contiguous()
        return self._pe_cache[key]

    def pre_loop(self, fmap1: torch.Tensor, fmap2: torch.Tensor, c4: torch.Tensor, c8: torch.Tensor, c16: torch.Tensor, t: int, ctx_ready=None):
        L.require_gpu(fmap1, fmap2, c4, c8, c16)
        lib, st = L.load(), L.stream_ptr
        N, C, h, w = fmap1.shape
        if C != 256 or h % 4 or w % 4:
            raise RuntimeError("pre_loop: 256-channel 1/4-resolution features with h, w multiples of 4 expected")
        dev = fmap1.device
        f32 = lambda *s: torch.empty(*s, dtype=torch.float32, device=dev)
        fm = [fmap1.contiguous().float(), fmap2.contiguous().float()]
        feats: Dict[str, torch.Tensor] = {"f1_4": fm[0], "f2_4": fm[1]}

        def mix(f, c, tag):
            c = c.contiguous().float()
            net, inp = f32(N, 128, f.shape[2], f.shape[3]), f32(N, 128, f.shape[2], f.shape[3])
            L.check(lib.ppms_ctx_mix(f.data_ptr(), c.data_ptr(), net.data_ptr(), inp.data_ptr(), N, f.shape[2] * f.shape[3], st()))
            feats["net_" + tag], feats["inp_" + tag] = net, inp

        h16, w16, h8, w8 = h // 4, w // 4, h // 2, w // 2
        f16 = []
        for f in fm:
            p = f32(N, C, h16, w16)
            L.check(lib.ppms_avgpool(f.data_ptr(), p.data_ptr(), N * C, h, w, 4, st()))
            f16.append(p)
        if self.sst is not None:
            f16 = list(self.sst(f16[0], f16[1], t))
        else:
            pe = self._pe(h16, w16, dev)
            for p in f16:
                L.check(lib.ppms_axpby(p.data_ptr(), pe.data_ptr(), p.data_ptr(), 1.0, 1.0, pe.numel(), p.numel(), st()))
        feats["f1_16"], feats["f2_16"] = f16
        if ctx_ready is not None:
            ctx_ready()
        mix(fm[0], c4, "4")
        mix(f16[0], c16, "16")
        for i, f in enumerate(fm):
            p = f32(N, C, h8, w8)
            L.check(lib.ppms_avgpool(f.data_ptr(), p.data_ptr(), N * C, h, w, 2, st()))
            q = bilinear(f16[i], (h8, w8), True)
            L.check(lib.ppms_axpby(p.data_ptr(), q.data_ptr(), p.data_ptr(), 0.5, 0.5, p.numel(), p.numel(), st()))
            feats[f"f{i + 1}_8"] = p
        mix(feats["f1_8"], c8, "8")
        return feats

    @torch.no_grad()
    def forward(self, image1: torch.Tensor, image2: torch.Tensor, flow_init=None, iters: int = 10, test_mode: bool = False, pipeline=None):
        if flow_init is not None:
            raise NotImplementedError("flow_init: the reference's own path for it reads undefined state (ppmstereo.py:691-693, 763)")
        if self.fnet is None or self.cnet is None:
            raise RuntimeError("PPMStereo.forward needs the encoders: pass fnet= / cnet= (outside the hot path, SURVEY.md section 8 f3-f5)")
        b, T, c, h, w = image1.shape
        if b != 1 and pipeline is not None:
            raise NotImplementedError("PPMStereo.forward: a ClipPipeline overlaps consecutive batch-1 clips")
        with torch.cuda.device(image1.device):
            im1 = (2 * (image1 / 255.0) - 1.0).contiguous().reshape(b * T, c, h, w)
            im2 = (2 * (image2 / 255.0) - 1.0).contiguous().reshape(b * T, c, h, w)
            cur = torch.cuda.current_stream(image1.device)
            if self.parallel_encoders:
                side = self._encoder_stream(image1.device)
                side.wait_stream(cur)
                im1.record_stream(side)
                with torch.cuda.stream(side):
                    c4, c8, c16 = self.cnet(im1)
                fmap1, fmap2 = self.fnet([im1, im2])
                for t_ in (c4, c8, c16):
                    if torch.is_tensor(t_):
                        t_.record_stream(cur)
                ready = {"done": False}

                def ctx_ready():
                    if not ready["done"]:
                        cur.wait_stream(side)
                        ready["done"] = True
            else:
                fmap1, fmap2 = self.fnet([im1, im2])
                c4, c8, c16 = self.cnet(im1)
                ctx_ready = None
            if b == 1:
                feats = self.pre_loop(fmap1, fmap2, c4, c8, c16, T, ctx_ready)
            else:
                if ctx_ready is not None:
                    ctx_ready()
                per = [self.pre_loop(*(x[bi * T:(bi + 1) * T] for x in (fmap1, fmap2, c4, c8, c16)), T) for bi in range(b)]
                feats = {k: torch.cat([p_[k] for p_ in per]) for k in per[0]}
            preds, uncs = [], []
            self.cascade(feats, iters, T, preds, uncs, test_mode=test_mode, pipeline=pipeline if test_mode else None)
            if test_mode:
                return preds[-1].reshape(b, T, 1, h, w), uncs[-1].reshape(b, T, 1, h, w)
            return torch.stack(preds).reshape(-1, b, T, 1, h, w), torch.stack(uncs).reshape(-1, b, T, 1, h, w)

    @torch.no_grad()
    def forward_batch_test(self, batch_dict: Dict, kernel_size: int = 20, iters: int = 20, device=None, shard_ranks: bool = False):
        video = batch_dict["stereo_video"]
        num_ims = len(video)
        dev = torch.device("cuda", torch.cuda.current_device()) if device is None else torch.device(device)
        disp_preds, uncertainties = [], []
        plan = window_plan(num_ims, kernel_size)
        if shard_ranks and torch.distributed.is_available() and torch.distributed.is_initialized():
            from . import dist as D
            rank, world = torch.distributed.get_rank(), torch.distributed.get_world_size()
            mine_d, mine_u, first = [], [], 0
            firsts = []
            for start, stop, keep_from, keep_to in plan:
                firsts.append(start + keep_from)
            for wi, (start, stop, keep_from, keep_to) in enumerate(plan):
                if wi % world != rank:
                    continue
                win = video[start:stop].to(dev)
                left, right = win[:, 0], win[:, 1]
                padder = InputPadder(left.shape, divis_by=32)
                left, right = padder.pad(left, right)
                d, u = self.forward(left[None], right[None], iters=iters, test_mode=True)
                d, u = padder.unpad(d[0]), padder.unpad(u[0])
                mine_d.append((firsts[wi], d[keep_from:keep_to].abs()[:, :1]))
                mine_u.append((firsts[wi], u[keep_from:keep_to].abs()[:, :1]))
            H0, W0 = video.shape[-2:]
            disp = D.gather_kept_frames(mine_d, num_ims, H0, W0)
            unc = D.gather_kept_frames(mine_u, num_ims, H0, W0)
            return {"disparity": disp.cpu(), "uncertainties": unc.cpu()}
        pipe = ClipPipeline(dev) if len(plan) > 1 else None
        pending = None

        def collect(item):
            d, u, handle, padder, keep_from, keep_to = item
            if pipe is not None:
                pipe.wait(handle)
            du = torch.cat([padder.unpad(d[0])[:, None], padder.unpad(u[0])[:, None]])
            torch.cuda.current_stream(du.device).synchronize()
            du = du.cpu()
            d, u = du[:du.shape[0] // 2], du[du.shape[0] // 2:]
            disp_preds.append(d[keep_from:keep_to])
            uncertainties.append(u[keep_from:keep_to])

        with torch.cuda.device(dev):
            for start, stop, keep_from, keep_to in plan:
                win = video[start:stop].to(dev)
                left, right = win[:, 0], win[:, 1]
                padder = InputPadder(left.shape, divis_by=32)
                left, right = padder.pad(left, right)
                d, u = self.forward(left[None], right[None], iters=iters, test_mode=True, pipeline=pipe)
                item = (d, u, None if pipe is None else pipe.last, padder, keep_from, keep_to)
                if pending is not None:
                    collect(pending)
                pending = item
            collect(pending)
        return {"disparity": torch.cat(disp_preds).squeeze(1).abs()[:, :1], "uncertainties": torch.cat(uncertainties).squeeze(1).abs()[:, :1]}


def window_plan(num_ims: int, kernel_size: int = 20):
    stride = kernel_size // 2
    if kernel_size > num_ims:
        return [(0, num_ims, 0, num_ims)]
    plan = []
    for i in range(0, num_ims, stride):
        n = min(i + kernel_size, num_ims) - i
        if plan and n >= stride:
            plan.append((i, i + n, stride // 2, n if n < kernel_size else n + (-stride // 2)))
        elif not plan:
            plan.append((i, i + n, 0, n + (-stride // 2)))
    return plan


def shard_windows(plan, rank: int, world: int):
    return [w for i, w in enumerate(plan) if i % world == rank]
```

### ppmstereo_amd/update.py

```python
from __future__ import annotations

import math
from collections import OrderedDict
from typing import Optional, Tuple

import torch
import torch.nn as nn

from . import _lib as L
from .convplan import CONV2, pack_conv
from .engine import PackedBlock, ScaleEngine, temporal_pe


@torch.no_grad()
def get_temporal_positional_encoding(max_sequence_len, channels, device, is_normalize=False, scale=2 * math.pi, is_debug=False):
    if is_normalize and scale == 1.0:
        pe = temporal_pe(max_sequence_len, channels)
    else:
        pos = torch.arange(max_sequence_len)
        if is_normalize:
            pos = pos / pos[-1] * scale
        pos = pos.unsqueeze(1)
        div = 1.0 / (10000.0 ** (torch.arange(0, channels, 2).float() / channels))
        ang = pos * div
        pe = torch.zeros(max_sequence_len, channels)
        pe[:, 0::2], pe[:, 1::2] = torch.sin(ang), torch.cos(ang)
    return pe.view(max_sequence_len, 1, 1, channels).to(device)


class _Holder(nn.Module):
    def forward(self, *a, **k):
        raise RuntimeError("parameter holder: the gfx950 engine runs this layer")


class _PCBlock(_Holder):

    def __init__(self, c_in, c_out, k_conv):
        super().__init__()
        self.conv_list = nn.ModuleList([nn.Conv2d(c_in, c_in, k, padding=k // 2, groups=c_in) for k in k_conv])
        mid = int(1.5 * c_in)
        self.ffn1 = nn.Sequential(nn.Conv2d(c_in, mid, 1), nn.GELU(), nn.Conv2d(mid, c_in, 1))
        self.pw = nn.Conv2d(c_in, c_in, 1)
        self.ffn2 = nn.Sequential(nn.Conv2d(c_in, mid, 1), nn.GELU(), nn.Conv2d(mid, c_out, 1))


class _MotionEncoder(_Holder):

    def __init__(self, cor_planes):
        super().__init__()
        self.convc1 = _PCBlock(cor_planes, 256, [1, 7])
        self.convc2 = nn.Conv2d(256, 192, 3, padding=1)
        self.convf1 = nn.Conv2d(2, 128, 7, padding=3)
        self.convf2 = nn.Conv2d(128, 64, 3, padding=1)
        self.final_conv = nn.Conv2d(320, 190, 3, padding=1)
        self.init_conv = nn.Sequential(nn.Conv2d(128, 64, 3, padding=1), nn.ReLU(inplace=True), nn.Conv2d(64, 64, 3, padding=1))


class _GRU(_Holder):

    def __init__(self, hidden_dim, input_dim):
        super().__init__()
        c = hidden_dim + input_dim
        two = lambda: nn.Sequential(nn.Conv3d(c, hidden_dim, (1, 1, 15), padding=(0, 0, 7)), nn.GELU(),
                                    nn.Conv3d(hidden_dim, hidden_dim, (1, 1, 5), padding=(0, 0, 2)))
        self.convz1, self.convr1 = two(), two()
        self.convq1 = nn.Conv3d(c, hidden_dim, (1, 1, 5), padding=(0, 0, 2))
        for n, k, p in (("2", (1, 5, 1), (0, 2, 0)), ("3", (5, 1, 1), (2, 0, 0))):
            for g in "zrq":
                setattr(self, f"conv{g}{n}", nn.Conv3d(c, hidden_dim, k, padding=p))


class _FlowHead(_Holder):
    def __init__(self, input_dim=128, hidden_dim=256):
        super().__init__()
        self.conv1 = nn.Conv3d(input_dim, hidden_dim, 3, padding=1)
        self.conv2 = nn.Conv3d(hidden_dim, 2, 3, padding=1)


class _Attention(_Holder):
    def __init__(self, dim):
        super().__init__()
        self.qkv = nn.Linear(dim, dim * 3, bias=False)
        self.proj = nn.Linear(dim, dim)


class _TimeAttn(_Holder):
    def __init__(self, dim):
        super().__init__()
        self.temporal_attn = _Attention(dim)
        self.temporal_fc = nn.Linear(dim, dim)
        self.temporal_norm1 = nn.LayerNorm(dim)
        nn.init.constant_(self.temporal_fc.weight, 0)
        nn.init.constant_(self.temporal_fc.bias, 0)


class _LoFTR(_Holder):
    def __init__(self, d):
        super().__init__()
        self.q_proj, self.k_proj, self.v_proj, self.merge = (nn.Linear(d, d, bias=False) for _ in range(4))
        self.mlp = nn.Sequential(nn.Linear(2 * d, 2 * d, bias=False), nn.ReLU(), nn.Linear(2 * d, d, bias=False))
        self.norm1, self.norm2 = nn.LayerNorm(d), nn.LayerNorm(d)


class _SpaceAttn(_Holder):
    def __init__(self, dim):
        super().__init__()
        self.encoder_layer = _LoFTR(dim)


class _Aggregate(_Holder):
    def __init__(self, dim=128):
        super().__init__()
        self.to_v = nn.Conv2d(dim, dim, 1, bias=False)
        self.beta = nn.Parameter(torch.zeros(1))


class Attention_qk(nn.Module):

    def __init__(self, *, num_heads=1, dim_head=128):
        super().__init__()
        if dim_head != 128:
            raise NotImplementedError("Attention_qk: dim_head must be 128")
        self.heads, self.scale = num_heads, dim_head ** -0.5
        self.to_qk = nn.Conv2d(dim_head, dim_head * 2, 1, bias=False)
        self._packed = None
        self.register_load_state_dict_post_hook(lambda m, k: setattr(m, "_packed", None))

    def packed(self, device):
        if self._packed is None or self._packed[CONV2][0].device != torch.device(device):
            self._packed = pack_conv(self.to_qk.weight.detach().to(device).float(), None, [128], kernels=(CONV2,))
        return self._packed

    def forward(self, fmap):
        raise RuntimeError("Attention_qk.forward is not on the hot path; forward_update_block projects q/k inside the engine")


class SequenceUpdateBlock3D(nn.Module):

    def __init__(self, hidden_dim, cor_planes, mask_size=8, use_convex_3d=False, attention_type=None):
        super().__init__()
        if hidden_dim != 128 or cor_planes != 36 or mask_size != 4:
            raise NotImplementedError("SequenceUpdateBlock3D: hidden_dim=128, cor_planes=36, mask_size=4 (the PPMStereo configuration)")
        self.encoder = _MotionEncoder(cor_planes)
        self.gru = _GRU(hidden_dim, 256 + hidden_dim)
        self.flow_head = _FlowHead(hidden_dim, 256)
        self.uncertainty = nn.Sequential(nn.Conv2d(hidden_dim + 128, hidden_dim, 3, padding=1), nn.ReLU(inplace=True),
                                         nn.Conv2d(hidden_dim, 1, 1), nn.Sigmoid())
        self.use_convex_3d = bool(use_convex_3d)
        if self.use_convex_3d:
            self.mask_3d = nn.Sequential(nn.Conv3d(hidden_dim, hidden_dim + 128, 3, padding=1), nn.ReLU(inplace=True),
                                         nn.Conv3d(hidden_dim + 128, (mask_size ** 2) * 27, 1, padding=0))
        else:
            self.mask_2d = nn.Sequential(nn.Conv2d(hidden_dim, hidden_dim + 128, 3, padding=1), nn.ReLU(inplace=True),
                                         nn.Conv2d(hidden_dim + 128, (mask_size ** 2) * 9, 1))
        self.attention_type = attention_type
        if attention_type is not None:
            if "update_time" in attention_type:
                self.time_attn = _TimeAttn(384)
            if "update_space" in attention_type:
                self.space_attn = _SpaceAttn(384)
            if not ("update_time" in attention_type and "update_space" in attention_type):
                raise NotImplementedError("attention_type must contain both update_time and update_space (or be None)")
        self.aggregator = _Aggregate(128)
        self._pk: Optional[PackedBlock] = None
        self._engines: "OrderedDict[Tuple, ScaleEngine]" = OrderedDict()
        self.register_load_state_dict_post_hook(lambda m, k: m.invalidate())

    MAX_ENGINES = 2

    def invalidate(self):
        self._pk = None
        self._engines = OrderedDict()

    def packed(self, device) -> PackedBlock:
        if self._pk is None or self._pk.beta.device != torch.device(device):
            sd = {k: v for k, v in self.state_dict().items()}
            with torch.cuda.device(device):
                self._pk = PackedBlock(sd, device)
            self._engines = OrderedDict()
        return self._pk

    def engine(self, T: int, h: int, w: int, device, shard=None, slot: int = 0) -> ScaleEngine:
        device = torch.device(device)
        if device.index is None:
            device = torch.device("cuda", torch.cuda.current_device())
        key = (T, h, w, str(device), None if shard is None else (shard.rank, shard.world, shard.T, id(shard.group), bool(getattr(shard, "force_comm", False))), slot)
        pk = self.packed(device)
        if key not in self._engines:
            while len(self._engines) >= max(self.MAX_ENGINES, slot + 1):
                self._engines.popitem(last=False)
            with torch.cuda.device(device):
                self._engines[key] = ScaleEngine(pk, T, h, w, device, shard)
        self._engines.move_to_end(key)
        eng = self._engines[key]
        if shard is not None and eng.shard is not None:
            eng.shard = shard
        return eng

    def get_motion_and_value(self, flow, corr, motion_hidden_state, inp):
        L.require_gpu(flow, corr, inp)
        N, _, h, w = flow.shape
        with torch.cuda.device(flow.device):
            e = self.engine(N, h, w, flow.device)
            e.set_flow(flow)
            e.set_inp(inp)
            e.set_mhs(motion_hidden_state)
            e.load_nchw(corr, e.CORR.view(0, 36))
            L.check(e.lib.ppms_f32_to_sp(e.FLOW.data_ptr(), 2, e.X.view(254, 2), e.P, L.stream_ptr()))
            e.motion_and_value()
            return e.get_mf(), e.get_mhs(), e.get_value()

    def get_uncertainty(self, net):
        L.require_gpu(net)
        N, c, h, w = net.shape
        if c != 256:
            raise RuntimeError("get_uncertainty expects cat([net, value]) with 256 channels")
        with torch.cuda.device(net.device):
            e = self.engine(N, h, w, net.device)
            e.set_net(net[:, :128])
            e.load_nchw(net[:, 128:], e.VAL.view())
            e.uncertainty()
            return e.get_unc()

    def forward(self, net, inp, motion_features, motion_features_global, t=1):
        L.require_gpu(net, inp, motion_features, motion_features_global)
        N, _, h, w = net.shape
        if N != t:
            raise NotImplementedError("batch size 1 only: the frame axis of the 3-D convolutions is the whole batch")
        with torch.cuda.device(net.device):
            e = self.engine(N, h, w, net.device)
            e.set_net(net)
            e.set_inp(inp)
            e.set_mf(motion_features)
            e.set_mfg(motion_features_global)
            e.update()
            return e.get_net(), e.get_mask(), e.get_dflow()
```

Measured before the change: 23.60 million disparity-px/s.

## Fuse corr lookup into chainA and depthwise 7x7 conv into chainB

Adds a corr_encoder entry point that folds the correlation pyramid lookup into the first pointwise chain kernel and the 7x7 depthwise GELU conv into the second chain kernel. This drops two separate launches, plus the HBM round trips for the CORR and C1 intermediates, at small scales (P <= 16384). Larger scales keep the old separate path. The trade-off is that the fused kernels recompute halos and reload weights per tile, and they add LDS pressure.

```diff
diff --git a/include/ppms.h b/include/ppms.h
--- a/include/ppms.h
+++ b/include/ppms.h
@@ -139,6 +139,9 @@
 int ppms_pwchain(const void* dev_params, int64_t pixels, void* stream);
 int ppms_pwchain_param_bytes(void);
 
+int ppms_corr_encoder(const void* chain_a, const void* chain_b, const float* const pyr[4], const float* flow, ppms_sp flow_out, ppms_sp x2,
+                      const float* w7t, const float* b7, int BT, int H, int W, void* stream);
+
 int ppms_time_attn(ppms_sp x, const float* ln_w, const float* ln_b, ppms_sp out, int T, int n, int heads, void* stream);
 int ppms_layernorm(const float* x, int ld, const float* w, const float* b, ppms_sp resid, ppms_sp out, int64_t pixels, int C, void* stream);
 int64_t ppms_linear_attention_workspace_floats(int T, int n, int heads, int dh);
diff --git a/ppmstereo_amd/_lib.py b/ppmstereo_amd/_lib.py
--- a/ppmstereo_amd/_lib.py
+++ b/ppmstereo_amd/_lib.py
@@ -113,6 +113,7 @@
     "ppms_attn_prep_k": (c_int, [c_void_p, c_int, c_void_p, c_void_p, c_void_p, c_void_p, c_int, c_int, c_int, c_void_p]),
     "ppms_pwchain": (c_int, [c_void_p, c_int64, c_void_p]),
     "ppms_pwchain_param_bytes": (c_int, []),
+    "ppms_corr_encoder": (c_int, [c_void_p, c_void_p, C.POINTER(c_void_p), c_void_p, SP, SP, c_void_p, c_void_p, c_int, c_int, c_int, c_void_p]),
     "ppms_time_attn": (c_int, [SP, c_void_p, c_void_p, SP, c_int, c_int, c_int, c_void_p]),
     "ppms_layernorm": (c_int, [c_void_p, c_int, c_void_p, c_void_p, SP, SP, c_int64, c_int, c_void_p]),
     "ppms_linear_attention_workspace_floats": (c_int64, [c_int, c_int, c_int, c_int]),
diff --git a/ppmstereo_amd/build.py b/ppmstereo_amd/build.py
--- a/ppmstereo_amd/build.py
+++ b/ppmstereo_amd/build.py
@@ -14,8 +14,8 @@
 LIB = os.path.join(HERE, "libppms.so")
 STAMP = LIB + ".stamp"
 LOCK = LIB + ".lock"
-SOURCES = ["corr.hip", "conv_gemm2.hip", "conv_gemm5.hip", "conv_gemm6.hip", "gemm1.hip", "conv_stream.hip", "small_ops.hip", "encoder_ops.hip", "mem_attn.hip", "attn16.hip", "pwchain.hip"]
-HEADERS = ["common.h", "corr_lookup.h", "conv_epilogue.h", "conv5_asm.h", "conv6_asm.h", "attn64_asm.h", os.path.join("..", "..", "include", "ppms.h")]
+SOURCES = ["corr.hip", "conv_gemm2.hip", "conv_gemm5.hip", "conv_gemm6.hip", "gemm1.hip", "conv_stream.hip", "small_ops.hip", "encoder_ops.hip", "mem_attn.hip", "attn16.hip", "pwchain.hip", "corr_encoder.hip"]
+HEADERS = ["common.h", "corr_lookup.h", "pwchain.h", "conv_epilogue.h", "conv5_asm.h", "conv6_asm.h", "attn64_asm.h", os.path.join("..", "..", "include", "ppms.h")]
 COMMON = ["--offload-arch=gfx950", "-O3", "-std=c++17", "-fPIC", "-ffp-contract=off", "-I" + os.path.join(ROOT, "include"), "-I" + CSRC]
 NO_PK = ["-Xclang", "-target-feature", "-Xclang", "-packed-fp32-ops"]
 EXTRA = [x for x in os.environ.get("PPMS_BUILD_DEFINES", "").split() if x]
diff --git a/ppmstereo_amd/csrc/corr_encoder.hip b/ppmstereo_amd/csrc/corr_encoder.hip
--- /dev/null
+++ b/ppmstereo_amd/csrc/corr_encoder.hip
@@ -0,0 +1,55 @@
+#include "pwchain.h"
+
+namespace {
+__global__ __launch_bounds__(256) void corr_enc_lookup_chain_kernel(const ChainParams* __restrict__ cp, EncArgs e) {
+    pwchain_body<STAGE_LOOKUP>(cp, e);
+}
+__global__ __launch_bounds__(256) void corr_enc_dw7_chain_kernel(const ChainParams* __restrict__ cp, EncArgs e) { pwchain_body<STAGE_DW7>(cp, e); }
+__global__ __launch_bounds__(256) void corr_enc_lookup_chain32_kernel(const ChainParams* __restrict__ cp, EncArgs e) {
+    pwchain32_body<STAGE_LOOKUP>(cp, e);
+}
+__global__ __launch_bounds__(256) void corr_enc_dw7_chain32_kernel(const ChainParams* __restrict__ cp, EncArgs e) {
+    pwchain32_body<STAGE_DW7>(cp, e);
+}
+}
+
+extern "C" int ppms_corr_encoder(const void* chain_a, const void* chain_b, const float* const pyr[4], const float* flow, ppms_sp flow_out,
+                                 ppms_sp x2, const float* w7t, const float* b7, int BT, int H, int W, void* stream) {
+    PPMS_REQUIRE(chain_a != nullptr && chain_b != nullptr && pyr != nullptr && flow != nullptr && w7t != nullptr && b7 != nullptr,
+                 "corr_encoder: missing operand");
+    PPMS_REQUIRE(BT > 0 && H > 0 && (W >> 3) >= 2, "corr_encoder: bad shape BT=%d H=%d W=%d (level 3 needs >= 2 columns)", BT, H, W);
+    PPMS_REQUIRE(x2.hi && x2.lo && x2.c >= DW_CH && x2.ld % 8 == 0 && flow_out.hi && flow_out.lo && flow_out.c >= 2,
+                 "corr_encoder: x2 needs >= 40 channels (ld a multiple of 8), the flow view 2");
+    static ppms_device_once once;
+    once.run([] {
+        (void)hipFuncSetAttribute((const void*)corr_enc_lookup_chain_kernel, hipFuncAttributeMaxDynamicSharedMemorySize, (int)PWCHAIN_LDS);
+        (void)hipFuncSetAttribute((const void*)corr_enc_dw7_chain_kernel, hipFuncAttributeMaxDynamicSharedMemorySize, (int)PWCHAIN_LDS);
+        (void)hipFuncSetAttribute((const void*)corr_enc_lookup_chain32_kernel, hipFuncAttributeMaxDynamicSharedMemorySize, (int)PWCHAIN32_LDS);
+        (void)hipFuncSetAttribute((const void*)corr_enc_dw7_chain32_kernel, hipFuncAttributeMaxDynamicSharedMemorySize, (int)PWCHAIN32_LDS);
+    });
+    EncArgs e{};
+    for (int l = 0; l < 4; ++l) e.pyr[l] = pyr[l];
+    e.flow = flow;
+    e.fl = flow_out;
+    e.x2 = x2;
+    e.w7t = w7t;
+    e.b7 = b7;
+    e.H = H;
+    e.W = W;
+    const int64_t P = (int64_t)BT * H * W;
+    hipStream_t s = (hipStream_t)stream;
+    if (P <= 16384) {
+        e.tiles_x = ceil_div(W, DwTile<TP32>::TW);
+        e.tiles_y = ceil_div(H, DwTile<TP32>::TH);
+        hipLaunchKernelGGL(corr_enc_lookup_chain32_kernel, dim3(ceil_div(P, TP32)), dim3(256), PWCHAIN32_LDS, s, (const ChainParams*)chain_a, e);
+        hipLaunchKernelGGL(corr_enc_dw7_chain32_kernel, dim3((unsigned)BT * e.tiles_y * e.tiles_x), dim3(256), PWCHAIN32_LDS, s,
+                           (const ChainParams*)chain_b, e);
+    } else {
+        e.tiles_x = ceil_div(W, DwTile<TP>::TW);
+        e.tiles_y = ceil_div(H, DwTile<TP>::TH);
+        hipLaunchKernelGGL(corr_enc_lookup_chain_kernel, dim3(ceil_div(P, TP)), dim3(256), PWCHAIN_LDS, s, (const ChainParams*)chain_a, e);
+        hipLaunchKernelGGL(corr_enc_dw7_chain_kernel, dim3((unsigned)BT * e.tiles_y * e.tiles_x), dim3(256), PWCHAIN_LDS, s,
+                           (const ChainParams*)chain_b, e);
+    }
+    return ppms_check_launch("corr_encoder");
+}
diff --git a/ppmstereo_amd/csrc/pwchain.h b/ppmstereo_amd/csrc/pwchain.h
--- /dev/null
+++ b/ppmstereo_amd/csrc/pwchain.h
@@ -0,0 +1,522 @@
+#pragma once
+#include "common.h"
+#include "corr_lookup.h"
+
+namespace {
+
+constexpr int STAGE_LOAD = 0, STAGE_LOOKUP = 1, STAGE_DW7 = 2;
+
+constexpr int TP = 128;
+constexpr int ROWB = 64;
+constexpr int ACT_PLANE = TP * ROWB;
+constexpr int ACT_BUF = 4 * ACT_PLANE;
+constexpr int W_BLK = 2 * 2 * 64 * 64;
+
+__device__ __forceinline__ int swzp(int row, int chunk) { return row * 64 + ((chunk ^ ((row >> 2) & 3)) << 4); }
+
+struct Layer {
+    const void* w;
+    const float* bias;
+    const float* post_s;
+    const float* post_t;
+    int M;
+    int n_valid;
+    int resid;
+};
+
+struct ChainParams {
+    ppms_sp in, out;
+    Layer layer[3];
+    int nlayers;
+    int64_t P;
+};
+
+constexpr int ENC_CH = 36;
+constexpr int DW_CH = 40;
+struct EncArgs {
+    const float* pyr[4];
+    const float* flow;
+    ppms_sp fl;
+    ppms_sp x2;
+    const float* w7t;
+    const float* b7;
+    int H, W;
+    int tiles_x, tiles_y;
+};
+
+template <int TPX> struct DwTile;
+template <> struct DwTile<128> { static constexpr int TH = 8, TW = 16; };
+template <> struct DwTile<32> { static constexpr int TH = 4, TW = 8; };
+
+template <int STAGE, int TPX>
+__device__ __forceinline__ int64_t tile_pixel(const ChainParams& c, const EncArgs& e, int px) {
+    if constexpr (STAGE != STAGE_DW7) {
+        const int64_t p = (int64_t)blockIdx.x * TPX + px;
+        return p < c.P ? p : -1;
+    } else {
+        constexpr int TH = DwTile<TPX>::TH, TW = DwTile<TPX>::TW;
+        const int tx = (int)(blockIdx.x % (unsigned)e.tiles_x);
+        const int rest = (int)(blockIdx.x / (unsigned)e.tiles_x);
+        const int ty = rest % e.tiles_y, f = rest / e.tiles_y;
+        const int y = ty * TH + px / TW, x = tx * TW + px % TW;
+        return (y < e.H && x < e.W) ? ((int64_t)f * e.H + y) * e.W + x : -1;
+    }
+}
+
+template <int STAGE, int TPX>
+__device__ __forceinline__ void stage_input(const ChainParams& c, const EncArgs& e, char* buf, char* scratch) {
+    constexpr int PLANE = TPX * ROWB;
+    const int tid = threadIdx.x;
+    if constexpr (STAGE == STAGE_LOAD) {
+        for (int q = tid; q < TPX * 8; q += 256) {
+            const int px = q >> 3, ch = q & 7;
+            const int64_t pix = tile_pixel<STAGE, TPX>(c, e, px);
+            u32x4 vh = {0, 0, 0, 0}, vl = {0, 0, 0, 0};
+            if (pix >= 0) {
+                vh = gload16((const bf16_t*)c.in.hi + pix * c.in.ld + ch * 8);
+                vl = gload16((const bf16_t*)c.in.lo + pix * c.in.ld + ch * 8);
+            }
+            const int off = (ch >> 2) * 2 * PLANE + swzp(px, ch & 3);
+            *(u32x4*)(buf + off) = vh;
+            *(u32x4*)(buf + PLANE + off) = vl;
+        }
+    } else if constexpr (STAGE == STAGE_LOOKUP) {
+        constexpr int NS = 256 / TPX, SL = (ENC_CH + NS - 1) / NS;
+        static_assert(NS * TPX == 256, "one pass over the tile");
+        {
+            const int px = tid % TPX, sl = tid / TPX;
+            const int64_t pix = tile_pixel<STAGE, TPX>(c, e, px);
+            float v[SL];
+            const float xs = pix >= 0 ? (float)(int)(pix % e.W) + e.flow[pix * 2] : 0.0f;
+#pragma unroll
+            for (int j = 0; j < SL; ++j) {
+                const int ch = sl * SL + j;
+                v[j] = 0.0f;
+                if (pix >= 0 && ch < ENC_CH) {
+                    const int lvl = ch / 9, kk = ch - lvl * 9;
+                    const int Wl = e.W >> lvl;
+                    v[j] = lookup_tap(e.pyr[lvl] + pix * Wl, Wl, xs, lvl, kk);
+                }
+            }
+#pragma unroll
+            for (int j = 0; j < SL; ++j) {
+                const int ch = sl * SL + j;
+                if (ch < ENC_CH) {
+                    bf16_t hh, ll;
+                    split_bf16(v[j], hh, ll);
+                    const int off = (ch >> 5) * 2 * PLANE + swzp(px, (ch & 31) >> 3) + (ch & 7) * 2;
+                    *(bf16_t*)(buf + off) = hh;
+                    *(bf16_t*)(buf + PLANE + off) = ll;
+                }
+            }
+        }
+        for (int q = tid; q < TPX * 4; q += 256) {
+            const int px = q >> 2, ch = ENC_CH + (q & 3);
+            bf16_t hh, ll;
+            split_bf16(0.0f, hh, ll);
+            const int off = (ch >> 5) * 2 * PLANE + swzp(px, (ch & 31) >> 3) + (ch & 7) * 2;
+            *(bf16_t*)(buf + off) = hh;
+            *(bf16_t*)(buf + PLANE + off) = ll;
+        }
+        for (int q = tid; q < TPX * 3; q += 256) {
+            const int px = q / 3, ch8 = 5 + q - px * 3;
+            const int off = (ch8 >> 2) * 2 * PLANE + swzp(px, ch8 & 3);
+            *(u32x4*)(buf + off) = (u32x4){0, 0, 0, 0};
+            *(u32x4*)(buf + PLANE + off) = (u32x4){0, 0, 0, 0};
+        }
+        for (int px = tid; px < TPX; px += 256) {
+            const int64_t pix = tile_pixel<STAGE, TPX>(c, e, px);
+            if (pix >= 0) {
+                bf16_t h, l;
+                split_bf16(e.flow[pix * 2], h, l);
+                ((bf16_t*)e.fl.hi)[pix * e.fl.ld] = h;
+                ((bf16_t*)e.fl.lo)[pix * e.fl.ld] = l;
+                split_bf16(e.flow[pix * 2 + 1], h, l);
+                ((bf16_t*)e.fl.hi)[pix * e.fl.ld + 1] = h;
+                ((bf16_t*)e.fl.lo)[pix * e.fl.ld + 1] = l;
+            }
+        }
+    } else {
+        constexpr int TH = DwTile<TPX>::TH, TW = DwTile<TPX>::TW, HH = TH + 6, HW = TW + 6;
+        constexpr int HROW = ENC_CH;
+        float* halo = (float*)scratch;
+        constexpr int NPP = TPX < 64 ? 64 : TPX, GPR = 256 / NPP, NPASS = (5 + GPR - 1) / GPR;
+        float* wl = halo + HH * HW * HROW;
+        static_assert((HH * HW * HROW + 49 * GPR * 8) * 4 <= 4 * PLANE + (TPX == 128 ? W_BLK : 4 * W_BLK), "halo + weights fit the free LDS");
+        const int tx = (int)(blockIdx.x % (unsigned)e.tiles_x);
+        const int rest = (int)(blockIdx.x / (unsigned)e.tiles_x);
+        const int ty = rest % e.tiles_y, f = rest / e.tiles_y;
+        const int y0 = ty * TH, x0 = tx * TW;
+        const int64_t fbase = (int64_t)f * e.H * e.W;
+        constexpr int NQ = HH * HW * 5, QR = (NQ + 255) / 256;
+        bf16x8 hq[QR], lq[QR];
+#pragma unroll
+        for (int i = 0; i < QR; ++i) {
+            const int q = tid + i * 256;
+            hq[i] = (bf16x8){0, 0, 0, 0, 0, 0, 0, 0};
+            lq[i] = (bf16x8){0, 0, 0, 0, 0, 0, 0, 0};
+            if (q < NQ) {
+                const int hp = q / 5, ch8 = q - hp * 5;
+                const int hy = hp / HW, hx = hp - hy * HW;
+                const int y = y0 - 3 + hy, x = x0 - 3 + hx;
+                if ((unsigned)y < (unsigned)e.H && (unsigned)x < (unsigned)e.W) {
+                    const int64_t pix = fbase + (int64_t)y * e.W + x;
+                    hq[i] = *(const bf16x8*)((const bf16_t*)e.x2.hi + pix * e.x2.ld + ch8 * 8);
+                    lq[i] = *(const bf16x8*)((const bf16_t*)e.x2.lo + pix * e.x2.ld + ch8 * 8);
+                }
+            }
+        }
+#pragma unroll
+        for (int i = 0; i < QR; ++i) {
+            const int q = tid + i * 256;
+            if (q < NQ) {
+                const int hp = q / 5, ch8 = q - hp * 5;
+                const bf16x8 h8 = hq[i], l8 = lq[i];
+                float* d = halo + hp * HROW + ch8 * 8;
+                *(f32x4*)d = (f32x4){join_bf16(h8[0], l8[0]), join_bf16(h8[1], l8[1]), join_bf16(h8[2], l8[2]), join_bf16(h8[3], l8[3])};
+                if (ch8 < 4) *(f32x4*)(d + 4) = (f32x4){join_bf16(h8[4], l8[4]), join_bf16(h8[5], l8[5]), join_bf16(h8[6], l8[6]), join_bf16(h8[7], l8[7])};
+            }
+        }
+        for (int pass = 0; pass < NPASS; ++pass) {
+            __syncthreads();
+            for (int q = tid; q < 49 * GPR * 2; q += 256) {
+                const int tap = q / (GPR * 2), k = q - tap * GPR * 2;
+                const int cw = pass * GPR * 8 + k * 4;
+                *(f32x4*)(wl + tap * GPR * 8 + k * 4) = cw < DW_CH ? gld<f32x4>(e.w7t + tap * DW_CH + cw) : (f32x4){0.0f, 0.0f, 0.0f, 0.0f};
+            }
+            __syncthreads();
+            const int u = pass * 256 + tid;
+            const int g = __builtin_amdgcn_readfirstlane(u / NPP), px = u % NPP;
+            if (g >= 5 || px >= TPX) continue;
+            const int c0 = g * 8, wo = (g - pass * GPR) * 8;
+            const int py = px / TW, pxx = px - py * TW;
+            const int yy0 = y0 + py;
+            float acc[8], xc[8];
+            {
+                const f32x4 b0 = gld<f32x4>(e.b7 + c0), b1 = gld<f32x4>(e.b7 + c0 + 4);
+#pragma unroll
+                for (int j = 0; j < 8; ++j) {
+                    acc[j] = j < 4 ? b0[j & 3] : b1[j & 3];
+                    xc[j] = 0.0f;
+                }
+            }
+            const bool inside = yy0 < e.H && x0 + pxx < e.W;
+#pragma unroll
+            for (int ky = 0; ky < 7; ++ky) {
+                const int yy = yy0 + ky - 3;
+                if ((unsigned)yy >= (unsigned)e.H) continue;
+#pragma unroll
+                for (int kx = 0; kx < 7; ++kx) {
+                    const float* hsrc = halo + ((py + ky) * HW + pxx + kx) * HROW + c0;
+                    float win[8];
+                    const f32x4 v0 = *(const f32x4*)hsrc;
+                    const f32x4 v1 = g < 4 ? *(const f32x4*)(hsrc + 4) : (f32x4){0.0f, 0.0f, 0.0f, 0.0f};
+#pragma unroll
+                    for (int j = 0; j < 8; ++j) win[j] = j < 4 ? v0[j & 3] : v1[j & 3];
+                    if (ky == 3 && kx == 3) {
+#pragma unroll
+                        for (int j = 0; j < 8; ++j) xc[j] = win[j];
+                    }
+                    const float* wt = wl + (ky * 7 + kx) * GPR * 8 + wo;
+                    const f32x4 w0 = *(const f32x4*)wt, w1 = *(const f32x4*)(wt + 4);
+#pragma unroll
+                    for (int j = 0; j < 8; ++j) acc[j] += (j < 4 ? w0[j & 3] : w1[j & 3]) * win[j];
+                }
+            }
+            bf16x8 oh = {0, 0, 0, 0, 0, 0, 0, 0}, ol = {0, 0, 0, 0, 0, 0, 0, 0};
+            if (inside) {
+#pragma unroll
+                for (int j = 0; j < 8; ++j) {
+                    bf16_t hi, lo;
+                    split_bf16(gelu_erf(xc[j] + acc[j]), hi, lo);
+                    oh[j] = hi;
+                    ol[j] = lo;
+                }
+            }
+            const int off = (g >> 2) * 2 * PLANE + swzp(px, g & 3);
+            *(bf16x8*)(buf + off) = oh;
+            *(bf16x8*)(buf + PLANE + off) = ol;
+        }
+        for (int q = tid; q < TPX * 3; q += 256) {
+            const int px = q / 3, ch8 = 5 + q - px * 3;
+            const int off = (ch8 >> 2) * 2 * PLANE + swzp(px, ch8 & 3);
+            *(u32x4*)(buf + off) = (u32x4){0, 0, 0, 0};
+            *(u32x4*)(buf + PLANE + off) = (u32x4){0, 0, 0, 0};
+        }
+    }
+}
+
+template <int STAGE>
+__device__ __forceinline__ void pwchain_body(const ChainParams* __restrict__ cp, const EncArgs& e) {
+    extern __shared__ __attribute__((aligned(16))) char smem[];
+    const ChainParams& c = *cp;
+    char* bufX = smem;
+    char* bufA = smem + ACT_BUF;
+    char* wsm = smem + 2 * ACT_BUF;
+    const int tid = threadIdx.x, lane = tid & 63, wave = tid >> 6;
+    const int r = lane & 31, h = lane >> 5;
+
+    u32x4 wreg[4];
+    auto load_w = [&](int l, int mblk) __attribute__((always_inline)) {
+        const Layer& Lw = c.layer[l];
+        const int mbs = Lw.M / 64;
+#pragma unroll
+        for (int i = 0; i < 4; ++i) {
+            const int q = tid + i * 256;
+            const int ks = q >> 9, rem = q & 511;
+            wreg[i] = gload16((const char*)Lw.w + ((int64_t)(ks * mbs + mblk) * 512 + rem) * 16);
+        }
+    };
+    if constexpr (STAGE == STAGE_LOAD) {
+        stage_input<STAGE, TP>(c, e, bufX, bufA);
+        load_w(0, 0);
+    } else {
+        load_w(0, 0);
+        stage_input<STAGE, TP>(c, e, bufX, bufA);
+    }
+    const char* src = bufX;
+    for (int l = 0; l < c.nlayers; ++l) {
+        const Layer& L = c.layer[l];
+        const bool last = (l == c.nlayers - 1);
+        char* dst = (src == bufX) ? bufA : bufX;
+        const int mblocks = L.M / 64;
+        for (int mblk = 0; mblk < mblocks; ++mblk) {
+            __syncthreads();
+#pragma unroll
+            for (int i = 0; i < 4; ++i) *(u32x4*)(wsm + (tid + i * 256) * 16) = wreg[i];
+            if (mblk + 1 < mblocks)
+                load_w(l, mblk + 1);
+            else if (l + 1 < c.nlayers)
+                load_w(l + 1, 0);
+            __syncthreads();
+            f32x16 acc[2];
+            acc[0] = (f32x16){0};
+            acc[1] = (f32x16){0};
+#pragma unroll
+            for (int ks = 0; ks < 2; ++ks) {
+#pragma unroll
+                for (int k16 = 0; k16 < 2; ++k16) {
+                    const int boff = ks * 2 * ACT_PLANE + swzp(wave * 32 + r, 2 * k16 + h);
+                    const bf16x8 bh = *(const bf16x8*)(src + boff);
+                    const bf16x8 bl = *(const bf16x8*)(src + ACT_PLANE + boff);
+#pragma unroll
+                    for (int mb = 0; mb < 2; ++mb) {
+                        const int aoff = ks * 8192 + swzp(mb * 32 + r, 2 * k16 + h);
+                        const bf16x8 ah = *(const bf16x8*)(wsm + aoff);
+                        const bf16x8 al = *(const bf16x8*)(wsm + 4096 + aoff);
+                        acc[mb] = __builtin_amdgcn_mfma_f32_32x32x16_bf16(al, bh, acc[mb], 0, 0, 0);
+                        acc[mb] = __builtin_amdgcn_mfma_f32_32x32x16_bf16(ah, bl, acc[mb], 0, 0, 0);
+                        acc[mb] = __builtin_amdgcn_mfma_f32_32x32x16_bf16(ah, bh, acc[mb], 0, 0, 0);
+                    }
+                }
+            }
+            const int px = wave * 32 + r;
+#pragma unroll
+            for (int mb = 0; mb < 2; ++mb)
+#pragma unroll
+                for (int g = 0; g < 4; ++g) {
+                    const int cl = mb * 32 + 8 * g + 4 * h;
+                    const int cg = mblk * 64 + cl;
+                    const f32x4 b4 = gld<f32x4>(L.bias + cg);
+                    float y[4];
+#pragma unroll
+                    for (int j = 0; j < 4; ++j) y[j] = acc[mb][4 * g + j] + b4[j];
+                    if (L.resid) {
+                        const int xo = (cl >> 5) * 2 * ACT_PLANE + swzp(px, (cl & 31) >> 3) + (cl & 7) * 2;
+                        const bf16x4 xh = *(const bf16x4*)(bufX + xo), xl = *(const bf16x4*)(bufX + ACT_PLANE + xo);
+#pragma unroll
+                        for (int j = 0; j < 4; ++j) y[j] += join_bf16(xh[j], xl[j]);
+                    }
+#pragma unroll
+                    for (int j = 0; j < 4; ++j) y[j] = gelu_erf(y[j]);
+                    if (L.post_s != nullptr) {
+                        const f32x4 s4 = gld<f32x4>(L.post_s + cg), t4 = gld<f32x4>(L.post_t + cg);
+#pragma unroll
+                        for (int j = 0; j < 4; ++j) y[j] = gelu_erf(y[j] + (y[j] * s4[j] + t4[j]));
+                    }
+                    bf16x4 oh, ol;
+#pragma unroll
+                    for (int j = 0; j < 4; ++j) {
+                        bf16_t hh = (bf16_t)0.0f, ll = (bf16_t)0.0f;
+                        if (cg + j < L.n_valid) split_bf16(y[j], hh, ll);
+                        oh[j] = hh;
+                        ol[j] = ll;
+                    }
+                    {
+                        const int xo = (cl >> 5) * 2 * ACT_PLANE + swzp(px, (cl & 31) >> 3) + (cl & 7) * 2;
+                        *(bf16x4*)(dst + xo) = oh;
+                        *(bf16x4*)(dst + ACT_PLANE + xo) = ol;
+                    }
+                }
+            if (last) {
+                __syncthreads();
+                for (int qd = tid; qd < TP * 16; qd += 256) {
+                    const int opx = qd >> 4, plane = (qd >> 3) & 1, ch = qd & 7;
+                    const int64_t opix = tile_pixel<STAGE, TP>(c, e, opx);
+                    const int ocg = mblk * 64 + ch * 8;
+                    if (opix >= 0 && ocg < L.n_valid) {
+                        const u32x4 v = *(const u32x4*)(dst + (ch >> 2) * 2 * ACT_PLANE + plane * ACT_PLANE + swzp(opx, ch & 3));
+                        bf16_t* op = (bf16_t*)(plane ? c.out.lo : c.out.hi) + opix * c.out.ld + ocg;
+                        if (ocg + 8 <= L.n_valid) {
+                            gstore16(op, v);
+                        } else {
+                            const bf16_t* ev = (const bf16_t*)&v;
+                            for (int j = 0; j < 8; ++j)
+                                if (ocg + j < L.n_valid) gst<bf16_t>(op + j, ev[j]);
+                        }
+                    }
+                }
+            }
+        }
+        src = dst;
+    }
+}
+
+constexpr int TP32 = 32;
+constexpr int ACT32_PLANE = TP32 * ROWB;
+constexpr int ACT32_BUF = 4 * ACT32_PLANE;
+constexpr int W32_MAX = 4 * W_BLK;
+
+template <int STAGE>
+__device__ __forceinline__ void pwchain32_body(const ChainParams* __restrict__ cp, const EncArgs& e) {
+    extern __shared__ __attribute__((aligned(16))) char smem[];
+    const ChainParams& c = *cp;
+    char* bufX = smem;
+    char* bufA = smem + ACT32_BUF;
+    char* wsm = smem + 2 * ACT32_BUF;
+    const int tid = threadIdx.x, lane = tid & 63, wave = tid >> 6;
+    const int r = lane & 31, h = lane >> 5;
+    if constexpr (STAGE == STAGE_LOAD)
+        stage_input<STAGE, TP32>(c, e, bufX, bufA);
+    u32x4 wreg[16];
+    auto load_w = [&](int l) __attribute__((always_inline)) {
+        const Layer& Lw = c.layer[l];
+        const int mbs = Lw.M / 64;
+#pragma unroll
+        for (int mblk = 0; mblk < 4; ++mblk)
+            if (mblk < mbs) {
+#pragma unroll
+                for (int i = 0; i < 4; ++i) {
+                    const int q = tid + i * 256;
+                    const int ks = q >> 9, rem = q & 511;
+                    wreg[mblk * 4 + i] = gload16((const char*)Lw.w + ((int64_t)(ks * mbs + mblk) * 512 + rem) * 16);
+                }
+            }
+    };
+    load_w(0);
+    if constexpr (STAGE != STAGE_LOAD)
+        stage_input<STAGE, TP32>(c, e, bufX, bufA);
+    const char* src = bufX;
+    for (int l = 0; l < c.nlayers; ++l) {
+        const Layer& L = c.layer[l];
+        const bool last = (l == c.nlayers - 1);
+        char* dst = (src == bufX) ? bufA : bufX;
+        const int mbs = L.M / 64, nrb = L.M / 32;
+        __syncthreads();
+#pragma unroll
+        for (int mblk = 0; mblk < 4; ++mblk)
+            if (mblk < mbs) {
+#pragma unroll
+                for (int i = 0; i < 4; ++i) *(u32x4*)(wsm + mblk * W_BLK + (tid + i * 256) * 16) = wreg[mblk * 4 + i];
+            }
+        if (l + 1 < c.nlayers) load_w(l + 1);
+        __syncthreads();
+        bf16x4 keep_h[2][4], keep_l[2][4];
+#pragma unroll
+        for (int it = 0; it < 2; ++it) {
+            const int rb = wave + 4 * it;
+            if (rb >= nrb) continue;
+            const int mblk = rb >> 1, mb = rb & 1;
+            f32x16 acc = (f32x16){0};
+#pragma unroll
+            for (int ks = 0; ks < 2; ++ks)
+#pragma unroll
+                for (int k16 = 0; k16 < 2; ++k16) {
+                    const int boff = ks * 2 * ACT32_PLANE + swzp(r, 2 * k16 + h);
+                    const bf16x8 bh = *(const bf16x8*)(src + boff), bl = *(const bf16x8*)(src + ACT32_PLANE + boff);
+                    const int aoff = mblk * W_BLK + ks * 8192 + swzp(mb * 32 + r, 2 * k16 + h);
+                    const bf16x8 ah = *(const bf16x8*)(wsm + aoff), al = *(const bf16x8*)(wsm + 4096 + aoff);
+                    acc = __builtin_amdgcn_mfma_f32_32x32x16_bf16(al, bh, acc, 0, 0, 0);
+                    acc = __builtin_amdgcn_mfma_f32_32x32x16_bf16(ah, bl, acc, 0, 0, 0);
+                    acc = __builtin_amdgcn_mfma_f32_32x32x16_bf16(ah, bh, acc, 0, 0, 0);
+                }
+#pragma unroll
+            for (int g = 0; g < 4; ++g) {
+                const int cl = mb * 32 + 8 * g + 4 * h;
+                const int cg = mblk * 64 + cl;
+                const f32x4 b4 = gld<f32x4>(L.bias + cg);
+                float y[4];
+#pragma unroll
+                for (int j = 0; j < 4; ++j) y[j] = acc[4 * g + j] + b4[j];
+                const int xo = (cl >> 5) * 2 * ACT32_PLANE + swzp(r, (cl & 31) >> 3) + (cl & 7) * 2;
+                if (L.resid) {
+                    const bf16x4 xh = *(const bf16x4*)(bufX + xo), xl = *(const bf16x4*)(bufX + ACT32_PLANE + xo);
+#pragma unroll
+                    for (int j = 0; j < 4; ++j) y[j] += join_bf16(xh[j], xl[j]);
+                }
+#pragma unroll
+                for (int j = 0; j < 4; ++j) y[j] = gelu_erf(y[j]);
+                if (L.post_s != nullptr) {
+                    const f32x4 s4 = gld<f32x4>(L.post_s + cg), t4 = gld<f32x4>(L.post_t + cg);
+#pragma unroll
+                    for (int j = 0; j < 4; ++j) y[j] = gelu_erf(y[j] + (y[j] * s4[j] + t4[j]));
+                }
+                bf16x4 oh, ol;
+#pragma unroll
+                for (int j = 0; j < 4; ++j) {
+                    bf16_t hh = (bf16_t)0.0f, ll = (bf16_t)0.0f;
+                    if (cg + j < L.n_valid) split_bf16(y[j], hh, ll);
+                    oh[j] = hh;
+                    ol[j] = ll;
+                }
+                if (last) {
+                    keep_h[it][g] = oh;
+                    keep_l[it][g] = ol;
+                } else {
+                    *(bf16x4*)(dst + xo) = oh;
+                    *(bf16x4*)(dst + ACT32_PLANE + xo) = ol;
+                }
+            }
+        }
+        if (last) {
+            __syncthreads();
+            const int rowb = L.M * 2 + 16;
+#pragma unroll
+            for (int it = 0; it < 2; ++it) {
+                const int rb = wave + 4 * it;
+                if (rb >= nrb) continue;
+#pragma unroll
+                for (int g = 0; g < 4; ++g) {
+                    const int cg = rb * 32 + 8 * g + 4 * h;
+                    *(bf16x4*)(wsm + r * rowb + cg * 2) = keep_h[it][g];
+                    *(bf16x4*)(wsm + TP32 * rowb + r * rowb + cg * 2) = keep_l[it][g];
+                }
+            }
+            __syncthreads();
+            const int cpr = L.M / 8;
+            for (int qd = tid; qd < TP32 * 2 * cpr; qd += 256) {
+                const int plane = qd / (TP32 * cpr), rem = qd - plane * TP32 * cpr;
+                const int opx = rem / cpr, ch = rem - opx * cpr;
+                const int64_t opix = tile_pixel<STAGE, TP32>(c, e, opx);
+                const int ocg = ch * 8;
+                if (opix >= 0 && ocg < L.n_valid) {
+                    const u32x4 v = *(const u32x4*)(wsm + plane * TP32 * rowb + opx * rowb + ocg * 2);
+                    bf16_t* op = (bf16_t*)(plane ? c.out.lo : c.out.hi) + opix * c.out.ld + ocg;
+                    if (ocg + 8 <= L.n_valid) {
+                        gstore16(op, v);
+                    } else {
+                        const bf16_t* ev = (const bf16_t*)&v;
+                        for (int j = 0; j < 8; ++j)
+                            if (ocg + j < L.n_valid) gst<bf16_t>(op + j, ev[j]);
+                    }
+                }
+            }
+        }
+        src = dst;
+    }
+}
+
+constexpr size_t PWCHAIN_LDS = 2 * ACT_BUF + W_BLK;
+constexpr size_t PWCHAIN32_LDS = 2 * ACT32_BUF + W32_MAX;
+
+}
diff --git a/ppmstereo_amd/csrc/pwchain.hip b/ppmstereo_amd/csrc/pwchain.hip
--- a/ppmstereo_amd/csrc/pwchain.hip
+++ b/ppmstereo_amd/csrc/pwchain.hip
@@ -1,332 +1,22 @@
-#include "common.h"
+#include "pwchain.h"
 
 namespace {
-
-constexpr int TP = 128;
-constexpr int ROWB = 64;
-constexpr int ACT_PLANE = TP * ROWB;
-constexpr int ACT_BUF = 4 * ACT_PLANE;
-constexpr int W_BLK = 2 * 2 * 64 * 64;
-
-__device__ __forceinline__ int swzp(int row, int chunk) { return row * 64 + ((chunk ^ ((row >> 2) & 3)) << 4); }
-
-struct Layer {
-    const void* w;
-    const float* bias;
-    const float* post_s;
-    const float* post_t;
-    int M;
-    int n_valid;
-    int resid;
-};
-
-struct ChainParams {
-    ppms_sp in, out;
-    Layer layer[3];
-    int nlayers;
-    int64_t P;
-};
-
-__global__ __launch_bounds__(256) void pwchain_kernel(const ChainParams* __restrict__ cp) {
-    extern __shared__ __attribute__((aligned(16))) char smem[];
-    const ChainParams& c = *cp;
-    char* bufX = smem;
-    char* bufA = smem + ACT_BUF;
-    char* wsm = smem + 2 * ACT_BUF;
-    const int tid = threadIdx.x, lane = tid & 63, wave = tid >> 6;
-    const int r = lane & 31, h = lane >> 5;
-    const int64_t p0 = (int64_t)blockIdx.x * TP;
-
-    for (int q = tid; q < TP * 8; q += 256) {
-        const int px = q >> 3, ch = q & 7;
-        const int64_t pix = p0 + px;
-        u32x4 vh = {0, 0, 0, 0}, vl = {0, 0, 0, 0};
-        if (pix < c.P) {
-            vh = gload16((const bf16_t*)c.in.hi + pix * c.in.ld + ch * 8);
-            vl = gload16((const bf16_t*)c.in.lo + pix * c.in.ld + ch * 8);
-        }
-        const int off = (ch >> 2) * 2 * ACT_PLANE + swzp(px, ch & 3);
-        *(u32x4*)(bufX + off) = vh;
-        *(u32x4*)(bufX + ACT_PLANE + off) = vl;
-    }
-    u32x4 wreg[4];
-    auto load_w = [&](int l, int mblk) __attribute__((always_inline)) {
-        const Layer& Lw = c.layer[l];
-        const int mbs = Lw.M / 64;
-#pragma unroll
-        for (int i = 0; i < 4; ++i) {
-            const int q = tid + i * 256;
-            const int ks = q >> 9, rem = q & 511;
-            wreg[i] = gload16((const char*)Lw.w + ((int64_t)(ks * mbs + mblk) * 512 + rem) * 16);
-        }
-    };
-    load_w(0, 0);
-    const char* src = bufX;
-    for (int l = 0; l < c.nlayers; ++l) {
-        const Layer& L = c.layer[l];
-        const bool last = (l == c.nlayers - 1);
-        char* dst = (src == bufX) ? bufA : bufX;
-        const int mblocks = L.M / 64;
-        for (int mblk = 0; mblk < mblocks; ++mblk) {
-            __syncthreads();
-#pragma unroll
-            for (int i = 0; i < 4; ++i) *(u32x4*)(wsm + (tid + i * 256) * 16) = wreg[i];
-            if (mblk + 1 < mblocks)
-                load_w(l, mblk + 1);
-            else if (l + 1 < c.nlayers)
-                load_w(l + 1, 0);
-            __syncthreads();
-            f32x16 acc[2];
-            acc[0] = (f32x16){0};
-            acc[1] = (f32x16){0};
-#pragma unroll
-            for (int ks = 0; ks < 2; ++ks) {
-#pragma unroll
-                for (int k16 = 0; k16 < 2; ++k16) {
-                    const int boff = ks * 2 * ACT_PLANE + swzp(wave * 32 + r, 2 * k16 + h);
-                    const bf16x8 bh = *(const bf16x8*)(src + boff);
-                    const bf16x8 bl = *(const bf16x8*)(src + ACT_PLANE + boff);
-#pragma unroll
-                    for (int mb = 0; mb < 2; ++mb) {
-                        const int aoff = ks * 8192 + swzp(mb * 32 + r, 2 * k16 + h);
-                        const bf16x8 ah = *(const bf16x8*)(wsm + aoff);
-                        const bf16x8 al = *(const bf16x8*)(wsm + 4096 + aoff);
-                        acc[mb] = __builtin_amdgcn_mfma_f32_32x32x16_bf16(al, bh, acc[mb], 0, 0, 0);
-                        acc[mb] = __builtin_amdgcn_mfma_f32_32x32x16_bf16(ah, bl, acc[mb], 0, 0, 0);
-                        acc[mb] = __builtin_amdgcn_mfma_f32_32x32x16_bf16(ah, bh, acc[mb], 0, 0, 0);
-                    }
-                }
-            }
-            const int px = wave * 32 + r;
-            const int64_t pix = p0 + px;
-#pragma unroll
-            for (int mb = 0; mb < 2; ++mb)
-#pragma unroll
-                for (int g = 0; g < 4; ++g) {
-                    const int cl = mb * 32 + 8 * g + 4 * h;
-                    const int cg = mblk * 64 + cl;
-                    const f32x4 b4 = gld<f32x4>(L.bias + cg);
-                    float y[4];
-#pragma unroll
-                    for (int j = 0; j < 4; ++j) y[j] = acc[mb][4 * g + j] + b4[j];
-                    if (L.resid) {
-                        const int xo = (cl >> 5) * 2 * ACT_PLANE + swzp(px, (cl & 31) >> 3) + (cl & 7) * 2;
-                        const bf16x4 xh = *(const bf16x4*)(bufX + xo), xl = *(const bf16x4*)(bufX + ACT_PLANE + xo);
-#pragma unroll
-                        for (int j = 0; j < 4; ++j) y[j] += join_bf16(xh[j], xl[j]);
-                    }
-#pragma unroll
-                    for (int j = 0; j < 4; ++j) y[j] = gelu_erf(y[j]);
-                    if (L.post_s != nullptr) {
-                        const f32x4 s4 = gld<f32x4>(L.post_s + cg), t4 = gld<f32x4>(L.post_t + cg);
-#pragma unroll
-                        for (int j = 0; j < 4; ++j) y[j] = gelu_erf(y[j] + (y[j] * s4[j] + t4[j]));
-                    }
-                    bf16x4 oh, ol;
-#pragma unroll
-                    for (int j = 0; j < 4; ++j) {
-                        bf16_t hh = (bf16_t)0.0f, ll = (bf16_t)0.0f;
-                        if (cg + j < L.n_valid) split_bf16(y[j], hh, ll);
-                        oh[j] = hh;
-                        ol[j] = ll;
-                    }
-                    {
-                        const int xo = (cl >> 5) * 2 * ACT_PLANE + swzp(px, (cl & 31) >> 3) + (cl & 7) * 2;
-                        *(bf16x4*)(dst + xo) = oh;
-                        *(bf16x4*)(dst + ACT_PLANE + xo) = ol;
-                    }
-                }
-            if (last) {
-                __syncthreads();
-                for (int qd = tid; qd < TP * 16; qd += 256) {
-                    const int opx = qd >> 4, plane = (qd >> 3) & 1, ch = qd & 7;
-                    const int64_t opix = p0 + opx;
-                    const int ocg = mblk * 64 + ch * 8;
-                    if (opix < c.P && ocg < L.n_valid) {
-                        const u32x4 v = *(const u32x4*)(dst + (ch >> 2) * 2 * ACT_PLANE + plane * ACT_PLANE + swzp(opx, ch & 3));
-                        bf16_t* op = (bf16_t*)(plane ? c.out.lo : c.out.hi) + opix * c.out.ld + ocg;
-                        if (ocg + 8 <= L.n_valid) {
-                            gstore16(op, v);
-                        } else {
-                            const bf16_t* e = (const bf16_t*)&v;
-                            for (int j = 0; j < 8; ++j)
-                                if (ocg + j < L.n_valid) gst<bf16_t>(op + j, e[j]);
-                        }
-                    }
-                }
-            }
-        }
-        src = dst;
-    }
-}
-
-constexpr int TP32 = 32;
-constexpr int ACT32_PLANE = TP32 * ROWB;
-constexpr int ACT32_BUF = 4 * ACT32_PLANE;
-constexpr int W32_MAX = 4 * W_BLK;
-
-__global__ __launch_bounds__(256) void pwchain32_kernel(const ChainParams* __restrict__ cp) {
-    extern __shared__ __attribute__((aligned(16))) char smem[];
-    const ChainParams& c = *cp;
-    char* bufX = smem;
-    char* bufA = smem + ACT32_BUF;
-    char* wsm = smem + 2 * ACT32_BUF;
-    const int tid = threadIdx.x, lane = tid & 63, wave = tid >> 6;
-    const int r = lane & 31, h = lane >> 5;
-    const int64_t p0 = (int64_t)blockIdx.x * TP32;
-    {
-        const int px = tid >> 3, ch = tid & 7;
-        const int64_t pix = p0 + px;
-        u32x4 vh = {0, 0, 0, 0}, vl = {0, 0, 0, 0};
-        if (pix < c.P) {
-            vh = gload16((const bf16_t*)c.in.hi + pix * c.in.ld + ch * 8);
-            vl = gload16((const bf16_t*)c.in.lo + pix * c.in.ld + ch * 8);
-        }
-        const int off = (ch >> 2) * 2 * ACT32_PLANE + swzp(px, ch & 3);
-        *(u32x4*)(bufX + off) = vh;
-        *(u32x4*)(bufX + ACT32_PLANE + off) = vl;
-    }
-    u32x4 wreg[16];
-    auto load_w = [&](int l) __attribute__((always_inline)) {
-        const Layer& Lw = c.layer[l];
-        const int mbs = Lw.M / 64;
-#pragma unroll
-        for (int mblk = 0; mblk < 4; ++mblk)
-            if (mblk < mbs) {
-#pragma unroll
-                for (int i = 0; i < 4; ++i) {
-                    const int q = tid + i * 256;
-                    const int ks = q >> 9, rem = q & 511;
-                    wreg[mblk * 4 + i] = gload16((const char*)Lw.w + ((int64_t)(ks * mbs + mblk) * 512 + rem) * 16);
-                }
-            }
-    };
-    load_w(0);
-    const char* src = bufX;
-    for (int l = 0; l < c.nlayers; ++l) {
-        const Layer& L = c.layer[l];
-        const bool last = (l == c.nlayers - 1);
-        char* dst = (src == bufX) ? bufA : bufX;
-        const int mbs = L.M / 64, nrb = L.M / 32;
-        __syncthreads();
-#pragma unroll
-        for (int mblk = 0; mblk < 4; ++mblk)
-            if (mblk < mbs) {
-#pragma unroll
-                for (int i = 0; i < 4; ++i) *(u32x4*)(wsm + mblk * W_BLK + (tid + i * 256) * 16) = wreg[mblk * 4 + i];
-            }
-        if (l + 1 < c.nlayers) load_w(l + 1);
-        __syncthreads();
-        bf16x4 keep_h[2][4], keep_l[2][4];
-#pragma unroll
-        for (int it = 0; it < 2; ++it) {
-            const int rb = wave + 4 * it;
-            if (rb >= nrb) continue;
-            const int mblk = rb >> 1, mb = rb & 1;
-            f32x16 acc = (f32x16){0};
-#pragma unroll
-            for (int ks = 0; ks < 2; ++ks)
-#pragma unroll
-                for (int k16 = 0; k16 < 2; ++k16) {
-                    const int boff = ks * 2 * ACT32_PLANE + swzp(r, 2 * k16 + h);
-                    const bf16x8 bh = *(const bf16x8*)(src + boff), bl = *(const bf16x8*)(src + ACT32_PLANE + boff);
-                    const int aoff = mblk * W_BLK + ks * 8192 + swzp(mb * 32 + r, 2 * k16 + h);
-                    const bf16x8 ah = *(const bf16x8*)(wsm + aoff), al = *(const bf16x8*)(wsm + 4096 + aoff);
-                    acc = __builtin_amdgcn_mfma_f32_32x32x16_bf16(al, bh, acc, 0, 0, 0);
-                    acc = __builtin_amdgcn_mfma_f32_32x32x16_bf16(ah, bl, acc, 0, 0, 0);
-                    acc = __builtin_amdgcn_mfma_f32_32x32x16_bf16(ah, bh, acc, 0, 0, 0);
-                }
-#pragma unroll
-            for (int g = 0; g < 4; ++g) {
-                const int cl = mb * 32 + 8 * g + 4 * h;
-                const int cg = mblk * 64 + cl;
-                const f32x4 b4 = gld<f32x4>(L.bias + cg);
-                float y[4];
-#pragma unroll
-                for (int j = 0; j < 4; ++j) y[j] = acc[4 * g + j] + b4[j];
-                const int xo = (cl >> 5) * 2 * ACT32_PLANE + swzp(r, (cl & 31) >> 3) + (cl & 7) * 2;
-                if (L.resid) {
-                    const bf16x4 xh = *(const bf16x4*)(bufX + xo), xl = *(const bf16x4*)(bufX + ACT32_PLANE + xo);
-#pragma unroll
-                    for (int j = 0; j < 4; ++j) y[j] += join_bf16(xh[j], xl[j]);
-                }
-#pragma unroll
-                for (int j = 0; j < 4; ++j) y[j] = gelu_erf(y[j]);
-                if (L.post_s != nullptr) {
-                    const f32x4 s4 = gld<f32x4>(L.post_s + cg), t4 = gld<f32x4>(L.post_t + cg);
-#pragma unroll
-                    for (int j = 0; j < 4; ++j) y[j] = gelu_erf(y[j] + (y[j] * s4[j] + t4[j]));
-                }
-                bf16x4 oh, ol;
-#pragma unroll
-                for (int j = 0; j < 4; ++j) {
-                    bf16_t hh = (bf16_t)0.0f, ll = (bf16_t)0.0f;
-                    if (cg + j < L.n_valid) split_bf16(y[j], hh, ll);
-                    oh[j] = hh;
-                    ol[j] = ll;
-                }
-                if (last) {
-                    keep_h[it][g] = oh;
-                    keep_l[it][g] = ol;
-                } else {
-                    *(bf16x4*)(dst + xo) = oh;
-                    *(bf16x4*)(dst + ACT32_PLANE + xo) = ol;
-                }
-            }
-        }
-        if (last) {
-            __syncthreads();
-            const int rowb = L.M * 2 + 16;
-#pragma unroll
-            for (int it = 0; it < 2; ++it) {
-                const int rb = wave + 4 * it;
-                if (rb >= nrb) continue;
-#pragma unroll
-                for (int g = 0; g < 4; ++g) {
-                    const int cg = rb * 32 + 8 * g + 4 * h;
-                    *(bf16x4*)(wsm + r * rowb + cg * 2) = keep_h[it][g];
-                    *(bf16x4*)(wsm + TP32 * rowb + r * rowb + cg * 2) = keep_l[it][g];
-                }
-            }
-            __syncthreads();
-            const int cpr = L.M / 8;
-            for (int qd = tid; qd < TP32 * 2 * cpr; qd += 256) {
-                const int plane = qd / (TP32 * cpr), rem = qd - plane * TP32 * cpr;
-                const int opx = rem / cpr, ch = rem - opx * cpr;
-                const int64_t opix = p0 + opx;
-                const int ocg = ch * 8;
-                if (opix < c.P && ocg < L.n_valid) {
-                    const u32x4 v = *(const u32x4*)(wsm + plane * TP32 * rowb + opx * rowb + ocg * 2);
-                    bf16_t* op = (bf16_t*)(plane ? c.out.lo : c.out.hi) + opix * c.out.ld + ocg;
-                    if (ocg + 8 <= L.n_valid) {
-                        gstore16(op, v);
-                    } else {
-                        const bf16_t* e = (const bf16_t*)&v;
-                        for (int j = 0; j < 8; ++j)
-                            if (ocg + j < L.n_valid) gst<bf16_t>(op + j, e[j]);
-                    }
-                }
-            }
-        }
-        src = dst;
-    }
-}
-
+__global__ __launch_bounds__(256) void pwchain_kernel(const ChainParams* __restrict__ cp) { pwchain_body<STAGE_LOAD>(cp, EncArgs{}); }
+__global__ __launch_bounds__(256) void pwchain32_kernel(const ChainParams* __restrict__ cp) { pwchain32_body<STAGE_LOAD>(cp, EncArgs{}); }
 }
 
 static int pwchain_launch(const void* dev_params, int64_t pixels, void* stream) {
-    constexpr size_t lds = 2 * ACT_BUF + W_BLK;
-    constexpr size_t lds32 = 2 * ACT32_BUF + W32_MAX;
     static ppms_device_once once;
     once.run([] {
-        (void)hipFuncSetAttribute((const void*)pwchain_kernel, hipFuncAttributeMaxDynamicSharedMemorySize, (int)(2 * ACT_BUF + W_BLK));
-        (void)hipFuncSetAttribute((const void*)pwchain32_kernel, hipFuncAttributeMaxDynamicSharedMemorySize, (int)(2 * ACT32_BUF + W32_MAX));
+        (void)hipFuncSetAttribute((const void*)pwchain_kernel, hipFuncAttributeMaxDynamicSharedMemorySize, (int)PWCHAIN_LDS);
+        (void)hipFuncSetAttribute((const void*)pwchain32_kernel, hipFuncAttributeMaxDynamicSharedMemorySize, (int)PWCHAIN32_LDS);
     });
     if (pixels <= 16384) {
-        hipLaunchKernelGGL(pwchain32_kernel, dim3(ceil_div(pixels, TP32)), dim3(256), lds32, (hipStream_t)stream, (const ChainParams*)dev_params);
+        hipLaunchKernelGGL(pwchain32_kernel, dim3(ceil_div(pixels, TP32)), dim3(256), PWCHAIN32_LDS, (hipStream_t)stream,
+                           (const ChainParams*)dev_params);
         return ppms_check_launch("pwchain");
     }
-    hipLaunchKernelGGL(pwchain_kernel, dim3(ceil_div(pixels, TP)), dim3(256), lds, (hipStream_t)stream, (const ChainParams*)dev_params);
+    hipLaunchKernelGGL(pwchain_kernel, dim3(ceil_div(pixels, TP)), dim3(256), PWCHAIN_LDS, (hipStream_t)stream, (const ChainParams*)dev_params);
     return ppms_check_launch("pwchain");
 }
 
diff --git a/ppmstereo_amd/engine.py b/ppmstereo_amd/engine.py
--- a/ppmstereo_amd/engine.py
+++ b/ppmstereo_amd/engine.py
@@ -182,10 +182,12 @@
         self._ev, self._ev_i = None, 0
         self._xa_halo = None
         self._x_hid = False
-        self.hbm = {"corr_lookup": TimedCall(self._lookup), "attn_prep_k": TimedCall(self._prep_k), "convex_upsample": TimedCall(self._upsample)}
+        self.hbm = {"attn_prep_k": TimedCall(self._prep_k), "convex_upsample": TimedCall(self._upsample)}
         self._side = torch.cuda.Stream(device=device)
         self._ev_fork, self._ev_join = torch.cuda.Event(), torch.cuda.Event()
         self._build_descriptors()
+        if not self.fused_enc:
+            self.hbm = {"corr_lookup": TimedCall(self.lookup), **self.hbm}
 
     def _halo_sp(self, tensors, k: int, async_op: bool = False):
         if self.shard is None:
@@ -215,12 +217,19 @@
         w = {k: self.pk.w[k][CONV2] for k in ("ffn1_0", "ffn1_2", "pw", "ffn2_0", "ffn2_2")}
         (w1, b1, _), (w7, b7, _) = self.pk.dw
         dw1 = (w1.reshape(64).contiguous(), b1)
-        o["chainA"] = PwChain(self.CORR.view(), self.C2.view(), [(w["ffn1_0"], 54, False, None), (w["ffn1_2"], 36, True, dw1)], self.P, [dw1[0]],
-                             device=self.dev)
-        o["chainB"] = PwChain(self.C1.view(), self.COR256.view(), [(w["pw"], 36, True, None), (w["ffn2_0"], 54, False, None),
-                                                                   (w["ffn2_2"], 256, False, None)], self.P, [], device=self.dev)
-        o["dw7"] = TimedCall(lambda: L.check(self.lib.ppms_dwconv_gelu(self.C2.view(0, 40), self.C1.view(0, 40), w7.data_ptr(), b7.data_ptr(), 7,
-                                                                        self.T, self.h, self.w, L.stream_ptr())))
+        self.enc = {}
+        self.enc["chainA"] = PwChain(self.CORR.view(), self.C2.view(), [(w["ffn1_0"], 54, False, None), (w["ffn1_2"], 36, True, dw1)], self.P,
+                                     [dw1[0]], device=self.dev)
+        self.enc["chainB"] = PwChain(self.C1.view(), self.COR256.view(), [(w["pw"], 36, True, None), (w["ffn2_0"], 54, False, None),
+                                                                          (w["ffn2_2"], 256, False, None)], self.P, [], device=self.dev)
+        self.enc["dw7"] = TimedCall(lambda: L.check(self.lib.ppms_dwconv_gelu(self.C2.view(0, 40), self.C1.view(0, 40), w7.data_ptr(), b7.data_ptr(), 7,
+                                                                     self.T, self.h, self.w, L.stream_ptr())))
+        self._w7t, self._b7 = w7[:40].t().contiguous(), b7
+        self.fused_enc = self.P <= 16384
+        if self.fused_enc:
+            o["corr_encoder"] = TimedCall(self._corr_encoder)
+        else:
+            o["chainA"], o["chainB"], o["dw7"] = self.enc["chainA"], self.enc["chainB"], self.enc["dw7"]
         o["convf1"] = self._conv("convf1", [self.PATCH.view()], k1, E(act=L.ACT_RELU, n_valid=128, out_sp=self.FLO1.view()))
         for par in (0, 1):
             cf, cf_next = self.CF[par], self.CF[1 - par]
@@ -394,13 +403,14 @@
         return self._qk_ops[key]
 
     def lookup(self):
-        self.hbm["corr_lookup"]()
-
-    def _lookup(self):
-        X = self.X
-        fl = X.view(254, 2)
+        fl = self.X.view(254, 2)
         L.check(self.lib.ppms_corr_lookup(self.pyr_ptrs, self.FLOW.data_ptr(), 1, None, self.CORR.view().hi, self.CORR.view().lo, 64,
                                           fl.hi, fl.lo, 384, self.T, self.h, self.w, self._s()))
+
+    def _corr_encoder(self):
+        L.check(self.lib.ppms_corr_encoder(self.enc["chainA"].dev.data_ptr(), self.enc["chainB"].dev.data_ptr(), self.pyr_ptrs, self.FLOW.data_ptr(),
+                                           self.X.view(254, 2), self.C2.view(), self._w7t.data_ptr(), self._b7.data_ptr(), self.T, self.h, self.w,
+                                           self._s()))
 
     def hbm_bytes(self) -> Dict[str, float]:
         T, n, w = self.T, self.n, self.w
@@ -417,7 +427,7 @@
         self._ev_join.record(self._side)
         torch.cuda.current_stream().wait_event(self._ev_join)
 
-    def motion_and_value(self):
+    def motion_and_value(self, from_corr: bool = False):
         o, par = self.op, self.parity
         with self._fork():
             L.check(self.lib.ppms_flow_patch7(self.FLOW.data_ptr(), self.PATCH.view(), self.T, self.h, self.w, self._s()))
@@ -427,9 +437,14 @@
             o["init0"]()
             o[f"init2_{par}"]()
             self.have_mhs = True
-        o["chainA"]()
-        o["dw7"]()
-        o["chainB"]()
+        if from_corr or not self.fused_enc:
+            if not from_corr:
+                self.hbm["corr_lookup"]()
+            self.enc["chainA"]()
+            self.enc["dw7"]()
+            self.enc["chainB"]()
+        else:
+            o["corr_encoder"]()
         o[f"convc2_{par}"]()
         self._join()
         o[f"final_{par}"]()
@@ -577,7 +592,6 @@
                                                   self.h, self.w, self._s()))
 
     def iterate(self, need_up: bool = True):
-        self.lookup()
         self.motion_and_value()
         self.uncertainty()
         self.pick()
diff --git a/ppmstereo_amd/ppmstereo.py b/ppmstereo_amd/ppmstereo.py
--- a/ppmstereo_amd/ppmstereo.py
+++ b/ppmstereo_amd/ppmstereo.py
@@ -118,7 +118,7 @@
         flow_out = None
         for _ in range(iters):
             for eng in engs:
-                eng.lookup(), eng.motion_and_value(), eng.uncertainty(), eng.pick()
+                eng.motion_and_value(), eng.uncertainty(), eng.pick()
             picked = [eng.SCORE.gather(1, eng.SEL[:, :k].long()) for eng in engs]
             mean_all = torch.stack([x.sum(1) for x in picked]).sum(0) / float(b * k)
             outs, uncs = [], []
diff --git a/ppmstereo_amd/update.py b/ppmstereo_amd/update.py
--- a/ppmstereo_amd/update.py
+++ b/ppmstereo_amd/update.py
@@ -207,7 +207,7 @@
             e.set_mhs(motion_hidden_state)
             e.load_nchw(corr, e.CORR.view(0, 36))
             L.check(e.lib.ppms_f32_to_sp(e.FLOW.data_ptr(), 2, e.X.view(254, 2), e.P, L.stream_ptr()))
-            e.motion_and_value()
+            e.motion_and_value(from_corr=True)
             return e.get_mf(), e.get_mhs(), e.get_value()
 
     def get_uncertainty(self, net):
```

Measured after the change: 23.61 million disparity-px/s, median of 3. Within noise of the previous version (+0.1%).
